# BoyBaykiller/IDKEngine

Measured on AMD Instinct MI355X. Metric: Mray/s (primary+1 bounce) at 1920x1080, 1M-tri scene, higher is better.
Workload: dtype f32

## Files before the change

### idkengine_amd/csrc/host_context.hpp

```cpp
#pragma once


struct DevBuf {
    void* p = nullptr; size_t bytes = 0;
    hipError_t ensure(size_t n) { if (n <= bytes && p) return hipSuccess; if (p) (void)hipFree(p); p = nullptr; bytes = 0; if (n == 0) return hipSuccess; hipError_t e = hipMalloc(&p, n); if (e == hipSuccess) bytes = n; return e; }
    void release() { if (p) (void)hipFree(p); p = nullptr; bytes = 0; }
    template <class T> T* as() const { return (T*)p; }
};

struct PinnedStage {
    char* host = nullptr; hipEvent_t ev[2] = {nullptr, nullptr}; int half = 0;
    template <class Fill> hipError_t stage(DevBuf& dst, size_t capacity, size_t bytes, hipStream_t st, Fill&& fill)
    {
        hipError_t e;
        if (!host) {
            if ((e = hipHostMalloc((void**)&host, 2 * capacity, hipHostMallocDefault)) != hipSuccess) return e;
            for (int i = 0; i < 2; i++) if ((e = hipEventCreateWithFlags(&ev[i], hipEventDisableTiming)) != hipSuccess) return e;
            half = 0;
        } else if ((e = hipEventSynchronize(ev[half])) != hipSuccess) return e;
        char* h = host + (size_t)half * capacity;
        fill(h);
        if ((e = dst.ensure(capacity)) != hipSuccess) return e;
        if ((e = hipMemcpyAsync(dst.p, h, bytes, hipMemcpyHostToDevice, st)) != hipSuccess) return e;
        if ((e = hipEventRecord(ev[half], st)) != hipSuccess) return e;
// ... 89 lines not shown
    void release() { if (host) (void)hipHostFree(host); host = nullptr; dev = nullptr; }
    template <class T> T* host_as() const { return (T*)host; }
    template <class T> T* dev_as() const { return (T*)dev; }
};
struct DerivedScene : derived::State {
    DevBuf wnodes, wleaf, wids, wpair, wcounts; std::vector<uint32_t> wNodeOff, wLeafOff;
    DevBuf pairNodes;
    DevBuf instRec;
    DevBuf itlas, imarks, ichunks; int itlasNeed = 1; uint32_t ichunkCount = 0;
    DevBuf entRec, braidBuf; bool itlasBraided = false; int itlasDepth = 0, itlasEntries = 0;
    MappedWords overlap; bool isieveWorth = false;
    int uniMode = 0; uint32_t uniBaseB = 0, uniRestoreIdx = 0;
    DevBuf unodes, utlas, uTabs, uniBuf, uniEntRec; bool uniEligible = false; int uniCap = 0, uniEntries = 0, uniDepth = 0; MappedWords uni;
    MappedWords pkStats; unsigned long long pkSeen[6] = {0, 0, 0, 0, 0, 0}; float pkCam[36] = {0}; int pkW = 0, pkRows = 0, pkBatch = 0; float pkLastLive = -1.0f;
    void release()
    {
        for (DevBuf* b : {&wnodes, &wleaf, &wids, &wpair, &wcounts, &pairNodes, &instRec, &itlas, &imarks, &ichunks, &entRec, &braidBuf, &unodes, &utlas, &uTabs, &uniBuf, &uniEntRec}) b->release();
        overlap.release(); uni.release(); pkStats.release(); valid = 0;
    }
};

struct DevOptions {
    int forceGeneric = 0;
    int noTileCull = 0;
    int noLeanPrimary = 0;
    int leafMin = 0;
    int grabUnitLog2 = 10, grabFixed = 0;
    int ldsPad = 0;
    int traceWaves = 0;
    int gridHint = 2;
    int deferLast = 1;
    int lastOcclusion = 1;
    int foldLast = 1;
    int graphProbe = 0;
    int gridMidWaves = 20;
    int gridRaysX4 = 6;
    int traceVariant = 0;
    int bvhTiming = 0, bvhSmall = 32;
    int advMin = 0;
    int poolMin = 12;
    int leafPool = -1;
    int splitScatter = 6;
    int queryScheduler = 1;
    int groupThreads = -1;
    int fused = 1;
    int fusedShadeMin = 16;
    int splitPeek = 64;
    int splitDonor = 1;
    int split = 1;
    int wide = 0;
    int wideCap = 0;
    int wideCount = 0;
    int genPixelMajor = 8;
    int bouncePixelMajor = 1;
    int genGroupMax = 16;
    int instSieve = 8;
    int instSieveOverlap = 50;
    int instTlas = 8;
    int instTlasOverlap = 10;
    int instBraid = 0;
    int instUnify = 4096;
    int instGeneral = 0;
    int uniRefill = 32;
    int instUnifyRadius = 15;
    int pairNodes = 1;
    int packet = 1;
// ... 34 lines not shown
    int sceneStack = 1;
    int hInst0Blas = 0;
    DerivedScene derived;
    DevBuf wtotals;
    std::vector<GpuBlasInstance> hInstances; std::vector<char> hXforms; uint64_t uniLaunches = 0;
    int verSlots = 1; size_t vbytes[VB_COUNT] = {0}, vstride[VB_COUNT] = {0}; int valloc[VB_COUNT] = {1, 1, 1, 1, 1}, vcur[VB_COUNT] = {0};
    uint64_t lastMask[VB_COUNT] = {0};
    uint8_t lastSlots[VB_COUNT] = {0}; bool lastMulti = false;
    DevBuf verTab; PinnedStage verStage;
    char* hStage = nullptr; hipEvent_t evStage[4] = {nullptr, nullptr, nullptr, nullptr}; int stageNext = 0;
    PinnedUpload skyStage;
    hipEvent_t evSky = nullptr;
    int (*groupFlushAll)(void* user) = nullptr;
    DevBuf pmList;
    DevBuf trRec, contFlag, blockSums, rayO, rayT, rayR, aovA, aovN, hit, hitCost, primHit, queue[2], keys[2], keysTmp, sortKeys, sortVals, contMask, waveCounts, counts, work, sortHist, counters64;
    DevBuf img[3];
    FrameProducts products;
    int presW = 0, presH = 0;
    int resultSource = 0;
    PinnedUpload denoiseStage;
    int denoiseInput = 0;
    DevBuf geomRays, geomHits;
    int noiseOn = 0;
    DevBuf camTab;
    int rowLimit = 0x7fffffff;
    idkpt_bounce_exchange_fn exchangeFn = nullptr; void* exchangeUser = nullptr;
    idkpt_band_exchange_fn bandExchangeFn = nullptr; void* bandExchangeUser = nullptr; DevBuf bandTab;
    idkpt_band_exchange_device_fn bandExchangeDevFn = nullptr; void* bandExchangeDevUser = nullptr;
    idkpt_stats stats;
    uint32_t* hCounts = nullptr; uint32_t* dCountsMirror = nullptr;
    bool sceneNested = false;
    bool sceneNoEmission = false;
    struct { bool valid = false, allHits = false; int j = 0, side = 0, B = 0; uint32_t total = 0, Npad = 0;
             bool occl = false, pm = false, fold = false; const uint32_t* list = nullptr; size_t ldsBytes = 0; uint32_t grid = 0; } defer;
    uint64_t occlLaunches = 0;
    uint64_t foldBatches = 0;
    DevBuf radSave, deferCount;
    bool countersDirty = true;
    uint32_t* hOverflow = nullptr; uint32_t* dOverflow = nullptr;
    int tlasNeed = 1;
    hipEvent_t evFrame[2] = {nullptr, nullptr};
    std::vector<hipEvent_t> evPool; size_t evUsed = 0;
    double traceMsAcc = 0.0; uint64_t traceLaunchesAcc = 0;
    int lastQueueSide = 0; int lastQueueCountSlot = 0; bool lastFast = false, lastNeedsRegen = false, lastTileClass = false ; int lastBatch = 1; Frame lastFrame;
    int maxBatch = 1; uint32_t Npad = 0; std::vector<PendingSample> pending; DevBuf bases, qwork; uint32_t* hBases = nullptr; uint32_t* dBasesMirror = nullptr;
    PinnedStage camStage;
    bool grouped = false, inGroupFlush = false; int groupIndex = 0;
    hipEvent_t* evBounce = nullptr;
    int (*groupExchange)(void* user, dev_ctx* member, int bounce, int samples, const uint32_t** outBases) = nullptr; void* groupUser = nullptr;
    struct BuilderScratch* bscratch = nullptr;
    struct PeerPolicy* peer = nullptr;
};

static hipEvent_t next_event(dev_ctx* ctx)
{
    if (ctx->evUsed == ctx->evPool.size()) { hipEvent_t e = nullptr; if (hipEventCreate(&e) != hipSuccess) return nullptr; ctx->evPool.push_back(e); }
    return ctx->evPool[ctx->evUsed++];
}
static void resolve_trace_events(dev_ctx* ctx)
{
    for (size_t i = 0; i + 1 < ctx->evUsed; i += 2) { float ms = 0.0f; if (hipEventElapsedTime(&ms, ctx->evPool[i], ctx->evPool[i + 1]) == hipSuccess) { ctx->traceMsAcc += ms; ctx->traceLaunchesAcc++; } }
    ctx->evUsed = 0;
}
#define TRACE_T0() do { if (ctx->timing) { hipEvent_t _e = next_event(ctx); if (_e) (void)hipEventRecord(_e, st); } } while (0)
#define TRACE_T1() do { if (ctx->timing) { hipEvent_t _e = next_event(ctx); if (_e) (void)hipEventRecord(_e, st); } } while (0)

static int fail(dev_ctx* c, int code, const std::string& msg) { if (c) { c->lastError = msg; if (c->errFn) c->errFn(c->errUser, (int32_t)code, c->lastError.c_str()); } return code; }
#define HIPC(expr) do { hipError_t _e = (expr); if (_e != hipSuccess) { (void)hipGetLastError(); return fail(ctx, IDKPT_ERR_HIP, std::string(#expr) + ": " + hipGetErrorString(_e)); } } while (0)
#define REQUIRE(cond, msg) do { if (!(cond)) return fail(ctx, IDKPT_ERR_INVALID_ARGUMENT, msg); } while (0)
// ... 26 lines not shown
```

### idkengine_amd/csrc/host_options.hpp

```cpp
#pragma once

static int32_t dev_SetOption(dev_ctx* ctx, const char* name, int32_t value)
{
    if (!ctx || !name) return IDKPT_ERR_INVALID_ARGUMENT;
    HIPC(hipSetDevice(ctx->device));
    FLUSH();
    DevOptions& o = ctx->opt;
    const std::string n(name);
    if (n == "force_generic") o.forceGeneric = value != 0;
    else if (n == "no_tile_cull") o.noTileCull = value != 0;
    else if (n == "no_lean_primary") o.noLeanPrimary = value != 0;
    else if (n == "leaf_min") o.leafMin = std::max(0, value);
    else if (n == "grab_unit_log2") o.grabUnitLog2 = value;
    else if (n == "grab_fixed") o.grabFixed = value;
    else if (n == "lds_pad") o.ldsPad = value;
    else if (n == "trace_waves") o.traceWaves = std::max(0, value);
    else if (n == "grid_hint") o.gridHint = std::max(0, value);
    else if (n == "grid_rays_x4") o.gridRaysX4 = std::max(0, value);
    else if (n == "grid_mid_waves") o.gridMidWaves = std::max(0, value);
    else if (n == "defer_last") o.deferLast = value != 0;
    else if (n == "last_occlusion") o.lastOcclusion = value != 0;
    else if (n == "fold_last") o.foldLast = value != 0;
    else if (n == "split") { REQUIRE(value >= 0 && value <= 3, "idkptSetDeveloperOption: split is 0..3"); o.split = value; }
    else if (n == "split_donor") o.splitDonor = value != 0;
    else if (n == "split_peek") o.splitPeek = std::max(1, value);
    else if (n == "split_scatter") o.splitScatter = std::min(6, std::max(0, value));
    else if (n == "query_scheduler") o.queryScheduler = value != 0;
    else if (n == "group_threads") o.groupThreads = value;
    else if (n == "fused") { REQUIRE(value >= 0 && value <= 2, "idkptSetDeveloperOption: fused is 0..2"); o.fused = value; }
    else if (n == "fused_shade_min") o.fusedShadeMin = std::min(64, std::max(1, value));
    else if (n == "leaf_pool") { REQUIRE(value >= -1 && value <= 7, "idkptSetDeveloperOption: leaf_pool is -1 (automatic) or a mask 0..7 (1: primary launches, 2: the first bounce, 4: later bounces)"); o.leafPool = value; }
    else if (n == "pool_min") o.poolMin = std::max(0, value);
    else if (n == "adv_min") o.advMin = std::min(64, std::max(0, value));
#ifdef IDKPT_DEVELOPER
    else if (n == "graph_probe") o.graphProbe = std::max(0, value);
#endif
    else if (n == "inst_tlas_overlap") { REQUIRE(value >= 0 && value <= 100, "idkptSetDeveloperOption: inst_tlas_overlap is a percentage"); FLUSH(); o.instTlasOverlap = value; ctx->derived.invalidate(derived::Cause::InstOption); }
    else if (n == "bounce_pixel_major") { REQUIRE(value >= 0 && value <= 2, "idkptSetDeveloperOption: bounce_pixel_major is 0..2"); o.bouncePixelMajor = value; }
    else if (n == "gen_group_max") { REQUIRE(value >= 1 && value <= 16, "idkptSetDeveloperOption: gen_group_max is 1..16"); o.genGroupMax = value; }
    else if (n == "gen_pixel_major") { REQUIRE(value >= 0, "idkptSetDeveloperOption: gen_pixel_major is >= 0"); o.genPixelMajor = value; }
    else if (n == "inst_sieve_overlap") { REQUIRE(value >= 0 && value <= 100, "idkptSetDeveloperOption: inst_sieve_overlap is a percentage"); FLUSH(); o.instSieveOverlap = value; ctx->derived.invalidate(derived::Cause::InstOption); }
    else if (n == "inst_sieve") { REQUIRE(value >= 0, "idkptSetDeveloperOption: inst_sieve is >= 0"); FLUSH(); o.instSieve = value; ctx->derived.invalidate(derived::Cause::InstOption); }
    else if (n == "inst_braid") { REQUIRE(value >= 0, "idkptSetDeveloperOption: inst_braid is >= 0"); FLUSH(); o.instBraid = value; ctx->derived.invalidate(derived::Cause::InstOption); }
    else if (n == "pair_nodes") { REQUIRE(value == 0 || value == 1, "idkptSetDeveloperOption: pair_nodes is 0 or 1"); o.pairNodes = value; }
    else if (n == "inst_general") { REQUIRE(value >= 0, "idkptSetDeveloperOption: inst_general is >= 0"); FLUSH(); o.instGeneral = value; ctx->derived.invalidate(derived::Cause::InstOption); }
    else if (n == "uni_refill") { REQUIRE(value == 16 || value == 32, "idkptSetDeveloperOption: uni_refill is 16 or 32"); o.uniRefill = value; }
    else if (n == "inst_unify_radius") { REQUIRE(value >= 1 && value <= 512, "idkptSetDeveloperOption: inst_unify_radius is 1-512"); FLUSH(); o.instUnifyRadius = value; ctx->derived.invalidate(derived::Cause::InstOption); }
    else if (n == "inst_unify") { REQUIRE(value >= 0, "idkptSetDeveloperOption: inst_unify is >= 0"); FLUSH(); o.instUnify = value; ctx->derived.invalidate(derived::Cause::InstOption); }
    else if (n == "inst_tlas") { REQUIRE(value >= 0, "idkptSetDeveloperOption: inst_tlas is >= 0"); FLUSH(); o.instTlas = value; ctx->derived.invalidate(derived::Cause::InstOption); }
    else if (n == "packet") { REQUIRE(value >= 0 && value <= 2, "idkptSetDeveloperOption: packet is 0..2"); o.packet = value; ctx->derived.packet_reprobe(); }
    else if (n == "packet_min_live") { REQUIRE(value >= 0 && value <= 100, "idkptSetDeveloperOption: packet_min_live is a percentage"); o.packetMinLive = value; ctx->derived.packet_reprobe(); }
    else if (n == "packet_waves") { REQUIRE(value >= 0 && value <= 32, "idkptSetDeveloperOption: packet_waves is 0 (default) or 1..32"); o.packetWaves = value; }
    else if (n == "wide") { REQUIRE(value >= 0 && value <= 1, "idkptSetDeveloperOption: wide is 0 or 1"); FLUSH(); o.wide = value; }
    else if (n == "wide_cap") { REQUIRE(value >= 0 && value <= 96, "idkptSetDeveloperOption: wide_cap is 0 (default) or 4..96 rows"); o.wideCap = value; }
    else if (n == "wide_count") o.wideCount = value != 0;
// ... 15 lines not shown
```

### idkengine_amd/csrc/host_readback.hpp

```cpp
#pragma once

static int32_t dev_DownloadFrame(dev_ctx* ctx, int32_t slot, int32_t image, float* rgba, size_t bytes)
{
    if (!ctx || !rgba) return IDKPT_ERR_INVALID_ARGUMENT;
    REQUIRE(image >= 0 && image < 3, "idkptDownloadFrame: bad image id");
    REQUIRE(slot >= 0 && slot < ctx->ringSize, "idkptDownloadFrame: slot outside the frame ring");
    size_t need = (size_t)ctx->W * ctx->rows * 16;
    REQUIRE(bytes == need && need > 0, "idkptDownloadFrame: bytes must equal localRows*width*16");
    HIPC(hipSetDevice(ctx->device));
    FLUSH_KEEP();
    HIPC(hipMemcpyAsync(rgba, image_ptr(ctx, image, slot), need, hipMemcpyDeviceToHost, ctx->stream));
    SYNC_CHECKED();
    return IDKPT_OK;
}

static int32_t dev_GetFrameDevicePtr(dev_ctx* ctx, int32_t slot, int32_t image, void** outPtr, size_t* outBytes)
{
    if (!ctx || !outPtr) return IDKPT_ERR_INVALID_ARGUMENT;
    REQUIRE(image >= 0 && image < 3, "idkptGetFrameDevicePtr: bad image id");
    REQUIRE(slot >= 0 && slot < ctx->ringSize, "idkptGetFrameDevicePtr: slot outside the frame ring");
    HIPC(hipSetDevice(ctx->device));
    FLUSH_KEEP();
    { int rc = check_overflow(ctx); if (rc) return rc; }
    *outPtr = image_ptr(ctx, image, slot);
// ... 80 lines not shown
    const bool have = ctx->lastFast && ctx->lastTileClass;
    const int32_t tx = have ? (ctx->lastFrame.W + 7) / 8 : 0, ty = have ? (ctx->lastFrame.rows + 7) / 8 : 0;
    const int32_t n = have ? (ctx->lastFrame.tilePerSample ? ctx->lastBatch : 1) : 0;
    *tilesX = tx; *tilesY = ty; *sets = n;
    if (!out) return IDKPT_OK;
    const size_t need = (size_t)n * tx * ty;
    REQUIRE(bytes == need, "idkptDownloadTileClasses: bytes must equal sets*tilesX*tilesY (call with out = NULL for the three numbers)");
    if (need) { REQUIRE(ctx->tileClass.bytes >= need, "idkptDownloadTileClasses: no classification is resident"); HIPC(hipMemcpyAsync(out, ctx->tileClass.p, need, hipMemcpyDeviceToHost, ctx->stream)); }
    SYNC_CHECKED();
    return IDKPT_OK;
}

static int32_t dev_GetStats(dev_ctx* ctx, idkpt_stats* out)
{
    if (!ctx || !out) return IDKPT_ERR_INVALID_ARGUMENT;
    HIPC(hipSetDevice(ctx->device));
    FLUSH_KEEP();
    SYNC_CHECKED();
    idkpt_stats s = ctx->stats;
    for (int j = 0; j < 16; j++) { const uint32_t* hb = ctx->hBases + (size_t)j * (MAX_BATCH + 1); s.LastAliveCounts[j] = (j >= 1 && j < ctx->st.RayDepth) ? hb[ctx->lastBatch] - hb[ctx->lastBatch - 1] : 0; }
    s.LastAliveCounts[0] = s.Frames ? (ctx->lastFast ? ctx->hCounts[MAX_DEPTH_SLOTS - 1] : (uint32_t)((size_t)ctx->W * ctx->rows)) : 0;
    s.LastFrameMs = 0.0f; s.LastTraceMs = 0.0f;
    if (ctx->timing && s.Frames > 0) { float ms = 0.0f; if (hipEventElapsedTime(&ms, ctx->evFrame[0], ctx->evFrame[1]) == hipSuccess) s.LastFrameMs = ms; }
    resolve_trace_events(ctx);
    s.TraceMsTotal = ctx->traceMsAcc; s.TraceLaunches = ctx->traceLaunchesAcc;
    s.LastTraceMs = s.TraceLaunches ? (float)(s.TraceMsTotal / (double)s.TraceLaunches) : 0.0f;
    uint64_t c[4] = {0, 0, 0, 0};
    HIPC(hipMemcpyAsync(c, ctx->counters64.p, 32, hipMemcpyDeviceToHost, ctx->stream)); HIPC(hipStreamSynchronize(ctx->stream));
    s.NodePairVisits = c[0]; s.TriangleTests = c[1];
    if (ctx->opt.traceVariant == 107 || ctx->opt.traceVariant == 113 || ctx->opt.traceVariant == 116 || ctx->opt.traceVariant == 213) { uint64_t d[16]; HIPC(hipMemcpyAsync(d, ctx->counters64.p, 128, hipMemcpyDeviceToHost, ctx->stream)); HIPC(hipStreamSynchronize(ctx->stream)); fprintf(stderr, "[idkpt prof] cycles refill %llu node %llu leaf %llu other %llu | refills %llu lanes %llu | nodeSteps %llu lanes %llu | leafPhases %llu lanes %llu | leafTests %llu leafTrips %llu\n", (unsigned long long)d[4], (unsigned long long)d[5], (unsigned long long)d[6], (unsigned long long)d[7], (unsigned long long)d[8], (unsigned long long)d[9], (unsigned long long)d[10], (unsigned long long)d[11], (unsigned long long)d[12], (unsigned long long)d[13], (unsigned long long)d[14], (unsigned long long)d[15]); }
    s.RaysTraced = s.PrimaryRays + c[2];
    if (ctx->wtotals.p) { uint64_t w[16]; HIPC(hipMemcpyAsync(w, ctx->wtotals.p, TOTALS_BYTES, hipMemcpyDeviceToHost, ctx->stream)); HIPC(hipStreamSynchronize(ctx->stream)); s.WideFlaggedRays = w[0]; s.WideNodeVisits = w[1]; s.WideLeafRecords = w[2]; s.WideTriangleTests = w[3]; s.InstTlasFlaggedRays = w[4];
        s.PacketFlaggedRays = w[8]; s.PacketPackets = w[9]; s.PacketNodeSteps = w[10]; s.PacketLiveLanes = w[11]; s.PacketRaysEntered = w[12]; s.PacketTriangleRounds = w[13]; }
    s.LastOcclusionLaunches = ctx->occlLaunches; s.LastFoldBatches = ctx->foldBatches;
    s.InstUnifiedLaunches = ctx->uniLaunches; s.InstUnifiedEntries = ctx->derived.holds(derived::UNI) ? (uint32_t)ctx->derived.uniEntries : 0u; s.InstUnifiedTopDepth = ctx->derived.holds(derived::UNI) ? (uint32_t)ctx->derived.uniDepth : 0u;
    *out = s;
    return IDKPT_OK;
}

static int32_t dev_ResetStats(dev_ctx* ctx)
{
    if (!ctx) return IDKPT_ERR_INVALID_ARGUMENT;
    HIPC(hipSetDevice(ctx->device));
    FLUSH_KEEP();
    HIPC(hipStreamSynchronize(ctx->stream));
    memset(&ctx->stats, 0, sizeof(ctx->stats)); ctx->uniLaunches = 0; ctx->occlLaunches = 0; ctx->foldBatches = 0;
    if (ctx->derived.pkStats.host) memset(ctx->derived.pkStats.host, 0, 64);
    for (int i = 0; i < 6; i++) ctx->derived.pkSeen[i] = 0;
    ctx->evUsed = 0; ctx->traceMsAcc = 0.0; ctx->traceLaunchesAcc = 0;
    memset(ctx->hCounts, 0, (MAX_DEPTH_SLOTS - 1) * 4);
    HIPC(hipMemsetAsync(ctx->counters64.p, 0, 128, ctx->stream)); if (ctx->wtotals.p) HIPC(hipMemsetAsync(ctx->wtotals.p, 0, TOTALS_BYTES, ctx->stream)); HIPC(hipStreamSynchronize(ctx->stream));
    return IDKPT_OK;
}

static int32_t dev_EnableCounters(dev_ctx* ctx, int32_t enable) { if (!ctx) return IDKPT_ERR_INVALID_ARGUMENT; ctx->counters = enable != 0; return IDKPT_OK; }
static int32_t dev_EnableTiming(dev_ctx* ctx, int32_t enable) { if (!ctx) return IDKPT_ERR_INVALID_ARGUMENT; ctx->timing = enable != 0; return IDKPT_OK; }

static int32_t dev_GetImageDevicePtr(dev_ctx* ctx, int32_t image, void** outPtr, size_t* outBytes)
{
    if (!ctx || !outPtr) return IDKPT_ERR_INVALID_ARGUMENT;
    REQUIRE(image >= 0 && image < 3 && ctx->W > 0, "idkptGetImageDevicePtr: bad image / no size");
    HIPC(hipSetDevice(ctx->device));
    FLUSH_KEEP();
    { int rc = check_overflow(ctx); if (rc) return rc; }
    *outPtr = image_ptr(ctx, image, ctx->curSlot);
    if (outBytes) *outBytes = (size_t)ctx->W * ctx->rows * 16;
    return IDKPT_OK;
}

static int32_t dev_SetStream(dev_ctx* ctx, void* hipStream)
{
    if (!ctx) return IDKPT_ERR_INVALID_ARGUMENT;
    HIPC(hipSetDevice(ctx->device));
    FLUSH();
    HIPC(hipStreamSynchronize(ctx->stream));
    if (hipStream) { if (ctx->ownStream && ctx->stream) (void)hipStreamDestroy(ctx->stream); ctx->stream = (hipStream_t)hipStream; ctx->ownStream = false; }
    else if (!ctx->ownStream) { HIPC(hipStreamCreateWithFlags(&ctx->stream, hipStreamNonBlocking)); ctx->ownStream = true; }
    return IDKPT_OK;
}
// ... 83 lines not shown
```

### idkengine_amd/csrc/host_schedule.hpp

```cpp
#pragma once

static DScene make_dscene(dev_ctx* ctx, const uint8_t* slots, bool multi)
{
    DScene s;
    auto at = [&](int b) -> char* { return multi ? (char*)vb_buf(ctx, b).p : vb_ptr(ctx, b, slots ? slots[b] : ctx->vcur[b]); };
    s.nodes = (const float4*)at(VB_NODES); s.tris = ctx->tris.as<uint4>(); s.triVerts = (const float4*)at(VB_TRIVERTS);
    s.descs = ctx->descs.as<GpuBlasDesc>(); s.instances = ctx->instances.as<GpuBlasInstance>(); s.instanceCount = ctx->instanceCount;
    s.tlas = (const float4*)at(VB_TLAS); s.tlasCount = ctx->tlasCount; s.vertices = (const uint4*)at(VB_VERTICES);
    s.instRec = nullptr;
    s.pairNodes = nullptr;
    s.meshes = ctx->meshes.as<GpuMesh>(); s.materials = ctx->materials.as<GpuMaterial>(); s.xforms = (const float4*)at(VB_XFORMS);
    s.lights = ctx->lights.as<GpuLight>(); s.lightCount = ctx->lightCount; s.sky = ctx->sky.as<float4>(); s.skySize = ctx->skySize;
    s.textures = ctx->texDescs.as<TexDesc>(); s.textureCount = ctx->textureCount; s.srgbLut = ctx->srgbLut.as<float>();
    s.overflow = ctx->dOverflow;
    s.ver = multi ? ctx->verTab.as<uint32_t>() : nullptr;
    return s;
}
static DScene make_dscene(dev_ctx* ctx) { return make_dscene(ctx, nullptr, false); }
static DScene make_dscene_last(dev_ctx* ctx) { return make_dscene(ctx, ctx->lastSlots, ctx->lastMulti); }

static float4* image_ptr(dev_ctx* ctx, int i, int slot) { return ctx->img[i].as<float4>() + (size_t)slot * ((size_t)ctx->W * ctx->rows); }

#define GRID_MID_RAYS 14000000u
#define SPLIT_MAX_RAYS 1500000u
static bool want_split(const dev_ctx* ctx, uint32_t prev, bool known, int samples)
{
    if (ctx->opt.split == 0) return false;
    if (ctx->opt.split >= 2) return true;
    return known && sparse_view(ctx, samples) && prev > 0u && prev < SPLIT_MAX_RAYS;
}
#define FUSED_MAX_RAYS 600000u
static bool want_fused(const dev_ctx* ctx, uint32_t prev, bool known, int samples)
{
    if (ctx->opt.fused == 0) return false;
    if (ctx->opt.fused >= 2) return true;
    return known && prev > 0u && prev < FUSED_MAX_RAYS && few_traversed(ctx, prev, std::max(1, samples));
}
static bool want_occlusion(const dev_ctx* ctx, const TracePlan& plan, bool readsOnlyHitOrMiss, bool split)
{
    return readsOnlyHitOrMiss && ctx->opt.lastOcclusion != 0 && !plan.fused && (plan.walk == Walk::Plain || plan.walk == Walk::Fast) && !(split && plan.splitOk)
           && !plan.multiVer && !plan.counting && !ctx->counters && (ctx->opt.traceVariant == 0 || ctx->opt.traceVariant == 100);
}
static bool want_fold(const dev_ctx* ctx, bool tookOccl) { return tookOccl && ctx->opt.foldLast != 0; }
static bool may_fold(const dev_ctx* ctx, bool deferLast, bool deferAllHits) { return deferLast && !deferAllHits && ctx->opt.lastOcclusion != 0 && ctx->opt.foldLast != 0; }
static uint32_t small_launch_grid(uint32_t fullGrid, uint32_t prev, int hintMul, int raysX4, uint32_t midGrid)
{
    if (prev == 0u || hintMul <= 0) return fullGrid;
    const uint32_t cap = std::max<uint32_t>(256u, (uint32_t)(((uint64_t)hintMul * prev + 63) / 64));
    uint32_t g = cap;
    if (raysX4 > 0) g = std::max<uint32_t>((uint32_t)(((uint64_t)prev * 4u / (uint32_t)raysX4 + 63) / 64), std::min<uint32_t>(cap, 1024u));
    if (midGrid > 0u && prev < GRID_MID_RAYS) g = std::min(g, midGrid);
    return std::min(fullGrid, std::min(g, cap));
}

struct Batch {
    dev_ctx* ctx; hipStream_t st; int B, depth; uint32_t N, Npad, total, gridTotal, scanBlocks;
    bool multiVer, fast, debug, capturing;
    Frame f; DScene s; TracePlan plan;
    RayBufs rays; HitBufs hits; TraceBufs tr, trNone;
    uint32_t* counts; uint32_t* bases ; uint32_t* work; uint64_t* counters; uint32_t* hostCounts; uint32_t* hostBases;
    unsigned long long* contMask; uint32_t* waveLocal ; uint32_t* blockSums; uint32_t* keysTmp;
    uint32_t* activeList; uint32_t* activeCount;
    uint32_t* pmList; uint32_t* pmCount; bool pmBounce;
    const uint8_t* tileClass; uint32_t midGrid, traceGrid;
    int side;
};
static const int BS = MAX_BATCH + 1;

static void batch_views(dev_ctx* ctx, Batch& b, int B, uint32_t Npad)
{
    b.ctx = ctx; b.st = ctx->stream; b.B = B; b.depth = ctx->st.RayDepth; b.N = (uint32_t)((size_t)ctx->W * ctx->rows); b.Npad = Npad; b.total = (uint32_t)B * Npad;
    b.gridTotal = (b.total + 255) / 256; b.scanBlocks = ((b.total + 63) / 64 + SCAN_WAVES_PER_BLOCK - 1) / SCAN_WAVES_PER_BLOCK;
    b.rays = {ctx->rayO.as<float4>(), ctx->rayT.as<float4>(), ctx->rayR.as<float4>(), ctx->aovA.as<float4>(), ctx->aovN.as<float4>(), ctx->contFlag.as<uint8_t>()}; b.hits = {ctx->hit.as<float4>(), ctx->hitCost.as<float>()};
    b.tr = {ctx->trRec.as<float4>(), nullptr, nullptr, ctx->deferCount.as<uint32_t>() + 1}; b.trNone = {nullptr, nullptr, nullptr, nullptr};
    b.counts = ctx->counts.as<uint32_t>(); b.bases = ctx->bases.as<uint32_t>(); b.work = ctx->work.as<uint32_t>(); b.counters = ctx->counters64.as<uint64_t>(); b.hostCounts = ctx->dCountsMirror; b.hostBases = ctx->dBasesMirror;
    b.contMask = ctx->contMask.as<unsigned long long>(); b.waveLocal = ctx->waveCounts.as<uint32_t>(); b.blockSums = ctx->blockSums.as<uint32_t>(); b.keysTmp = ctx->keysTmp.as<uint32_t>();
    b.activeList = ctx->sortVals.as<uint32_t>(); b.activeCount = b.counts + (MAX_DEPTH_SLOTS - 1);
    b.pmList = nullptr; b.pmCount = b.counts + (MAX_DEPTH_SLOTS - 2); b.pmBounce = false; b.tileClass = nullptr; b.side = 1; b.capturing = false;
}

static int bounce_tail(Batch& b, int j, const uint32_t* q, const uint32_t* cnt, const uint32_t* gbase, unsigned long long* traced, bool record, const TraceBufs& tr)
{
    dev_ctx* ctx = b.ctx; hipStream_t st = b.st; const int side = b.side;
    with_flag(b.multiVer, [&](auto VER) { launch(k_shade<false, VER>, dim3(b.gridTotal), dim3(256), 0, st, b.s, b.f, b.rays, tr, b.hits, q, cnt, 0u, b.bases + j * BS, gbase, b.contMask, b.waveLocal, b.keysTmp); });
    launch(k_scan_local<false>, dim3(b.scanBlocks), dim3(SCAN_WAVES_PER_BLOCK), 0, st, cnt, 0u, nullptr, b.contMask, b.waveLocal, b.blockSums);
    launch(k_scan_blocks, dim3(1), dim3(1024), 0, st, cnt, 0u, b.blockSums, b.waveLocal, b.counts + j + 1, traced, b.contMask, b.bases + j * BS, b.Npad, b.B, b.bases + (j + 1) * BS, b.hostCounts + j + 1, b.hostBases + (size_t)(j + 1) * BS, nullptr, nullptr);
    if (record) HIPC(hipEventRecord(ctx->evBounce[j + 1], st));
    launch(k_compact<false>, dim3(b.gridTotal), dim3(256), 0, st, q, cnt, 0u, b.contMask, b.waveLocal, b.blockSums, b.keysTmp, ctx->queue[1 - side].as<uint32_t>(), ctx->keys[1 - side].as<uint32_t>());
    return IDKPT_OK;
}

static int finish_deferred(dev_ctx* ctx)
{
    if (!ctx->defer.valid) return IDKPT_OK;
    ctx->defer.valid = false;
    Batch b; batch_views(ctx, b, ctx->defer.B, ctx->defer.Npad);
    b.side = ctx->defer.side; b.f = ctx->lastFrame; b.f.markLast = 0; b.f.foldLast = 0; b.s = make_dscene_last(ctx); b.multiVer = ctx->lastMulti;
    const uint32_t* q = ctx->queue[b.side].as<uint32_t>(); const uint32_t* cnt = ctx->deferCount.as<uint32_t>();
    if (ctx->defer.occl) {
        const int j = ctx->defer.j;
        if (ctx->countersDirty) HIPC(hipMemsetAsync(b.work, 0, WORK_WORDS * 4, b.st));
        TracePlan p{}; p.walk = Walk::Plain; p.ldsBytes = ctx->defer.ldsBytes; p.grid = ctx->defer.grid;
        Frame ft = b.f; if (ctx->defer.pm) ft.hitsByRid = 0;
        if (ctx->defer.pm) launch_trace2<true>(ctx, p, p.grid, b.st, b.s, ft, b.rays, b.tr, b.hits, ctx->defer.list, cnt, b.work + j, b.counters, false, j);
        else launch_trace2<false>(ctx, p, p.grid, b.st, b.s, ft, b.rays, b.tr, b.hits, q, cnt, b.work + j, b.counters, false, j);
        ctx->defer.occl = false;
    }
    with_flag(ctx->defer.allHits, [&](auto ALL) { launch(k_restore_last<ALL>, dim3(b.gridTotal), dim3(256), 0, b.st, b.rays, b.hits, q, cnt, ctx->radSave.as<float4>(), b.f.hitsByRid, ctx->defer.fold ? 1 : 0); });
    { int rc = bounce_tail(b, ctx->defer.j, q, cnt, nullptr, nullptr, false, b.tr); if (rc) return rc; }
    HIPC(hipGetLastError());
    ctx->lastQueueSide = 1 - b.side; ctx->countersDirty = true;
    return IDKPT_OK;
}

static int stage_versions_cameras(Batch& b)
{
    dev_ctx* ctx = b.ctx; const int B = b.B;
    bool multiVer = false; for (int k = 1; k < B && !multiVer; k++) multiVer = memcmp(ctx->pending[k].vs, ctx->pending[0].vs, VB_COUNT) != 0;
    for (int v = 0; v < VB_COUNT; v++) { uint64_t m = 0; for (int k = 0; k < B; k++) m |= 1ull << ctx->pending[k].vs[v]; ctx->lastMask[v] = m; ctx->lastSlots[v] = ctx->pending[0].vs[v]; }
    ctx->lastMulti = b.multiVer = multiVer;
    auto fillVersions = [&](char* half) {
        for (int k = 0; k < B; k++) {
            const uint8_t* vs = ctx->pending[k].vs; uint32_t* row = (uint32_t*)half + (size_t)k * SCENE_VER_WORDS;
            for (int v = 0; v < VB_COUNT; v++) row[v] = (uint32_t)(((size_t)vs[v] * ctx->vstride[v]) / 16);
            for (int v = VB_COUNT; v < SCENE_VER_WORDS; v++) row[v] = 0u;
        } };
    if (multiVer) HIPC(ctx->verStage.stage(ctx->verTab, (size_t)MAX_BATCH * SCENE_VER_WORDS * 4, (size_t)B * SCENE_VER_WORDS * 4, b.st, fillVersions));
    b.s = make_dscene_last(ctx);
    memset(&b.f, 0, sizeof(b.f));
    if (ctx->ringSize > 1) {
        auto fillCameras = [&](char* half) { for (int k = 0; k < B; k++) memcpy(half + (size_t)k * 36 * 4, ctx->pending[k].cam, 36 * 4); };
// ... 5 lines not shown

#ifdef IDKPT_DEVELOPER
static void graph_probe_begin(Batch& b) { if (b.ctx->opt.graphProbe > 0 && !b.ctx->timing) b.capturing = hipStreamBeginCapture(b.st, hipStreamCaptureModeThreadLocal) == hipSuccess; }
static void graph_probe_end(Batch& b)
{
    if (!b.capturing) return;
    dev_ctx* ctx = b.ctx; hipStream_t st = b.st;
    hipGraph_t g = nullptr; hipGraphExec_t ex = nullptr; const int K = ctx->opt.graphProbe; ctx->opt.graphProbe = 0;
    if (hipStreamEndCapture(st, &g) == hipSuccess && g && hipGraphInstantiate(&ex, g, nullptr, nullptr, 0) == hipSuccess) {
        hipEvent_t e0 = nullptr, e1 = nullptr; (void)hipEventCreate(&e0); (void)hipEventCreate(&e1);
        (void)hipGraphLaunch(ex, st); (void)hipStreamSynchronize(st);
        (void)hipEventRecord(e0, st);
        for (int k = 0; k < K; k++) (void)hipGraphLaunch(ex, st);
        (void)hipEventRecord(e1, st); (void)hipStreamSynchronize(st);
        float ms = 0.0f; (void)hipEventElapsedTime(&ms, e0, e1);
        size_t nodes = 0; (void)hipGraphGetNodes(g, nullptr, &nodes);
        fprintf(stderr, "[idkpt graph] batch of %d sample(s) captured: %zu graph nodes; %d replays: %.1f us per batch\n", b.B, nodes, K, ms * 1000.0f / (float)K);
        (void)hipEventDestroy(e0); (void)hipEventDestroy(e1); (void)hipGraphExecDestroy(ex);
    } else fprintf(stderr, "[idkpt graph] capture or instantiation failed: %s\n", hipGetErrorString(hipGetLastError()));
    if (g) (void)hipGraphDestroy(g);
}
#else
static void graph_probe_begin(Batch&) {}
static void graph_probe_end(Batch&) {}
#endif

static int frame_setup(Batch& b)
{
    dev_ctx* ctx = b.ctx; hipStream_t st = b.st; Frame& f = b.f; const int B = b.B;
    memcpy(f.invProj, ctx->pending[0].cam, 64); memcpy(f.invView, ctx->pending[0].cam + 16, 64); memcpy(f.viewPos, ctx->pending[0].cam + 32, 12);
    f.W = ctx->W; f.H = ctx->H; f.rowMod = ctx->rowMod; f.rowRem = ctx->rowRem; f.rows = ctx->rows; f.rowBandLog2 = ctx->rowBandLog2;
    f.g = ctx->st.Gpu; f.useTlas = ctx->st.UseTlas; f.stackCap = std::max(1, ctx->st.BlasStackSize > 0 ? ctx->st.BlasStackSize : ctx->sceneStack);
    f.outputAovs = ctx->st.OutputAOVs; f.batch = B; f.Npad = b.Npad;
    HIPC(ctx->trRec.ensure((size_t)ctx->maxBatch * b.Npad * 64)); b.tr.rec = ctx->trRec.as<float4>();
    for (int k = 0; k < MAX_BATCH; k++) { f.accum[k] = k < B ? ctx->pending[k].accum : 0u; f.slotOf[k] = (uint32_t)(k < B ? ctx->pending[k].slot : 0); }
    f.seqFirst = ctx->seqFirst; f.seqStride = ctx->seqStride; f.accumulated = f.seqFirst + f.accum[0] * f.seqStride;
    f.tilePerSample = (f.cams != nullptr || b.multiVer) ? 1 : 0;
    graph_probe_begin(b);
    if (ctx->timing) HIPC(hipEventRecord(ctx->evFrame[0], st));
    ctx->defer.valid = false;
    if (ctx->countersDirty) { HIPC(hipMemsetAsync(b.work, 0, WORK_WORDS * 4, st)); HIPC(hipMemsetAsync(b.counts, 0, MAX_DEPTH_SLOTS * 4, st)); HIPC(hipMemsetAsync(b.tr.oddCount, 0, 4, st)); }
    ctx->countersDirty = true;
    f.tlasCap = std::min(TLAS_STACK_SIZE, std::max(1, ctx->tlasNeed));
    f.grabUnitLog2 = std::min(24, std::max(6, ctx->opt.grabUnitLog2)); f.grabFixed = std::max(0, ctx->opt.grabFixed);
    f.leafMin = ctx->opt.leafMin > 0 ? ctx->opt.leafMin : (B >= 4 ? 16 : 12);
    b.fast = fast_path(ctx);
    f.genPixelMajor = (b.fast && ctx->opt.genPixelMajor > 0 && B >= ctx->opt.genPixelMajor && !f.tilePerSample) ? 1 : 0;
    { int rc = trace_plan(ctx, f, b.s, b.multiVer, false, false, b.plan); if (rc) { ctx->pending.clear(); return rc; } }
    b.traceGrid = std::min<uint32_t>(b.plan.grid, std::max<uint32_t>(1u, (uint32_t)(((size_t)B * b.N + 63) / 64)));
    b.midGrid = (ctx->opt.gridMidWaves > 0 && ctx->opt.traceWaves == 0) ? (uint32_t)(ctx->numCUs * std::min(b.plan.wavesPerCU, ctx->opt.gridMidWaves)) : 0u;
    f.gridRaysX4 = (uint32_t)std::max(0, ctx->opt.gridRaysX4); f.gridMid = b.midGrid; f.gridMidRays = GRID_MID_RAYS; f.splitMode = (ctx->opt.split == 3 ? 2 : 1) | (ctx->opt.splitDonor ? 4 : 0); f.poolMin = ctx->opt.poolMin; f.advMin = ctx->opt.advMin > 0 ? ctx->opt.advMin : (B >= 4 ? 8 : 1); f.splitPeek = ctx->opt.splitPeek;
    b.debug = f.g.DoDebugBVHTraversal != 0; f.shadeMin = ctx->opt.fusedShadeMin; f.scatterLog2 = ctx->opt.splitScatter;
    if (!b.fast && (B != 1 || b.multiVer)) { ctx->pending.clear(); return fail(ctx, IDKPT_ERR_UNKNOWN, "internal: generic path is never batched"); }
    return IDKPT_OK;
}

static int first_hit_compact(Batch& b)
{
    dev_ctx* ctx = b.ctx; hipStream_t st = b.st;
    launch(k_scan_blocks, dim3(1), dim3(1024), 0, st, nullptr, b.total, b.blockSums, b.waveLocal, b.counts + 1, (unsigned long long*)(1 < b.depth ? b.counters + 2 : nullptr), b.contMask, nullptr, b.Npad, b.B, b.bases + 1 * BS, b.hostCounts + 1, b.hostBases + 1 * BS, b.counts + MAX_DEPTH_SLOTS - 1, b.hostCounts + MAX_DEPTH_SLOTS - 1);
    if (ctx->evBounce) HIPC(hipEventRecord(ctx->evBounce[1], st));
    launch(k_compact<true>, dim3(b.gridTotal), dim3(256), 0, st, nullptr, nullptr, b.total, b.contMask, b.waveLocal, b.blockSums, b.keysTmp, ctx->queue[1].as<uint32_t>(), ctx->keys[1].as<uint32_t>());
    return IDKPT_OK;
}

static int first_hit_fast(Batch& b)
{
    dev_ctx* ctx = b.ctx; hipStream_t st = b.st; Frame& f = b.f; const DScene& s = b.s; const int B = b.B; const uint32_t N = b.N;
    const uint32_t tilesX = ((uint32_t)f.W + 7) / 8, tilesY = ((uint32_t)f.rows + 7) / 8; const uint32_t genWaves = tilesX * tilesY;
    const int cull = f.g.DoTraceLights ? 0 : 1;
    const int lean = (cull && !f.useTlas && s.instanceCount == 1 && ctx->opt.noLeanPrimary == 0) ? 1 : 0;
    uint8_t* contFlag = ctx->contFlag.as<uint8_t>();
    if (ctx->capturePrimary) launch(k_fill_miss, dim3((N + 255) / 256), dim3(256), 0, st, b.hits, (size_t)(B - 1) * b.Npad, N);
    if (cull && !ctx->opt.noTileCull) {
        const uint32_t classSets = f.tilePerSample ? (uint32_t)B : 1u;
        HIPC(ctx->tileClass.ensure((size_t)genWaves * classSets));
        with_flag(b.multiVer, [&](auto VER) { launch(k_classify_tiles<VER>, dim3((genWaves + 255) / 256, classSets), dim3(256), 0, st, s, f, ctx->tileClass.as<uint8_t>(), tilesX, tilesY); });
        b.tileClass = ctx->tileClass.as<uint8_t>();
    }
    const int genMax = std::min(16, std::max(1, ctx->opt.genGroupMax)), genGroups = (B + genMax - 1) / genMax, genPer = (B + genGroups - 1) / genGroups;
    const dim3 genGrid = f.genPixelMajor ? dim3(genGroups, genWaves) : dim3(B, (genWaves + 15) / 16), genBlock = f.genPixelMajor ? dim3(64 * genPer) : dim3(1024);
    with_flag(b.multiVer, [&](auto VER) { launch(k_gen_primary<VER>, genGrid, genBlock, 0, st, s, f, b.rays, b.tr, cull, b.activeList, b.activeCount, b.keysTmp, contFlag, b.tileClass, lean); });
    TRACE_T0();
    const bool known = ctx->lastFast && ctx->lastBatch == B;
    uint32_t grid0 = b.traceGrid;
    if (ctx->opt.gridRaysX4 > 0 && known) grid0 = small_launch_grid(b.traceGrid, ctx->hCounts[MAX_DEPTH_SLOTS - 1], 2, ctx->opt.gridRaysX4, b.midGrid);
    if (b.plan.fused) launch(k_trace_fused<32>, dim3(grid0), dim3(WAVE), b.plan.ldsBytes, st, s, f, b.rays, b.tr, b.hits, b.activeList, b.activeCount, b.work + 0, contFlag, b.keysTmp, lean);
    else launch_trace2<true>(ctx, b.plan, grid0, st, s, f, b.rays, b.tr, b.hits, b.activeList, b.activeCount, b.work + 0, b.counters, want_split(ctx, ctx->hCounts[MAX_DEPTH_SLOTS - 1], known, B), 0);
    TRACE_T1();
    if (ctx->capturePrimary) { HIPC(ctx->primHit.ensure((size_t)N * 16)); launch(k_capture_primary, dim3((N + 255) / 256), dim3(256), 0, st, b.hits, (size_t)(B - 1) * b.Npad, N, ctx->primHit.as<float4>()); }
    if (!b.plan.fused) {
        const bool sparseView = ctx->lastFast && ctx->lastBatch >= 1 && few_traversed(ctx, ctx->hCounts[MAX_DEPTH_SLOTS - 1], ctx->lastBatch);
        b.pmBounce = f.genPixelMajor && (ctx->opt.bouncePixelMajor >= 2 || (ctx->opt.bouncePixelMajor == 1 && sparseView)) && b.depth >= 2 && !b.multiVer;
        if (b.pmBounce) { HIPC(ctx->pmList.ensure((size_t)b.total * 4)); b.pmList = ctx->pmList.as<uint32_t>(); }
        with_flag(b.multiVer, [&](auto VER) { launch(k_shade_first<VER>, dim3(b.gridTotal), dim3(256), 0, st, s, f, b.rays, b.tr, b.hits, b.activeList, b.activeCount, contFlag, b.keysTmp, lean, b.pmList, VER ? nullptr : b.pmCount); });
    }
    launch(k_scan_local<true>, dim3(b.scanBlocks), dim3(SCAN_WAVES_PER_BLOCK), 0, st, nullptr, b.total, contFlag, b.contMask, b.waveLocal, b.blockSums);
    return first_hit_compact(b);
}

static int first_hit_generic(Batch& b)
{
    dev_ctx* ctx = b.ctx; hipStream_t st = b.st; const uint32_t N = b.N;
    TRACE_T0();
    const uint32_t g = std::min<uint32_t>(b.traceGrid, (N + 63) / 64);
    with_flags(ctx->counters, b.debug, [&](auto COUNT, auto COST) { launch(k_trace_primary<COUNT, COST>, dim3(g), dim3(WAVE), b.plan.ldsBytes, st, b.s, b.f, b.rays, b.hits, N, b.work + 0, b.counters); });
    TRACE_T1();
    if (ctx->capturePrimary) { HIPC(ctx->primHit.ensure((size_t)N * 16)); launch(k_capture_primary, dim3((N + 255) / 256), dim3(256), 0, st, b.hits, 0, N, ctx->primHit.as<float4>()); }
    launch(k_shade<true, false>, dim3(b.gridTotal), dim3(256), 0, st, b.s, b.f, b.rays, b.trNone, b.hits, nullptr, nullptr, b.total, nullptr, nullptr, b.contMask, b.waveLocal, b.keysTmp);
    launch(k_scan_local<false>, dim3(b.scanBlocks), dim3(SCAN_WAVES_PER_BLOCK), 0, st, nullptr, b.total, nullptr, b.contMask, b.waveLocal, b.blockSums);
    return first_hit_compact(b);
}

static int exchange_bases(Batch& b, int j, const uint32_t* q, const uint32_t*& gbase)
{
    dev_ctx* ctx = b.ctx; hipStream_t st = b.st; Frame& f = b.f; const int B = b.B;
    gbase = nullptr; f.gbStride = 1; f.gbBands = 0;
    const bool bandExchange = (ctx->bandExchangeFn || ctx->bandExchangeDevFn) && ctx->rowMod > 1 && !(ctx->st.DoRaySorting && j > 1);
    if (!bandExchange && ctx->groupExchange) {
        const int rc = ctx->groupExchange(ctx->groupUser, ctx, j, B, &gbase); if (rc) ctx->pending.clear(); return rc; }
    if (!bandExchange && ctx->exchangeFn) {
        std::vector<uint32_t> hb(B + 1), local(B), outBases(B, 0u);
        HIPC(hipMemcpyAsync(hb.data(), b.bases + j * BS, (size_t)(B + 1) * 4, hipMemcpyDeviceToHost, st)); HIPC(hipStreamSynchronize(st));
        for (int b2 = 0; b2 < B; b2++) local[b2] = hb[b2 + 1] - hb[b2];
        ctx->exchangeFn(ctx->exchangeUser, j, B, local.data(), outBases.data());
        HIPC(ctx->gbases.ensure((size_t)MAX_BATCH * 4));
        HIPC(hipMemcpyAsync(ctx->gbases.p, outBases.data(), (size_t)B * 4, hipMemcpyHostToDevice, st)); HIPC(hipStreamSynchronize(st));
        gbase = ctx->gbases.as<uint32_t>();
    }
// ... 12 lines not shown
    } else {
        std::vector<uint32_t> starts((size_t)B * (LB + 1)), local((size_t)B * LB), outBases((size_t)B * LB, 0u), tab((size_t)B * LB);
        HIPC(hipMemcpyAsync(starts.data(), dStarts, starts.size() * 4, hipMemcpyDeviceToHost, st)); HIPC(hipStreamSynchronize(st));
        for (int k2 = 0; k2 < B; k2++) for (int b2 = 0; b2 < LB; b2++) local[(size_t)k2 * LB + b2] = starts[(size_t)k2 * (LB + 1) + b2 + 1] - starts[(size_t)k2 * (LB + 1) + b2];
        ctx->bandExchangeFn(ctx->bandExchangeUser, j, B, LB, local.data(), outBases.data());
        for (int k2 = 0; k2 < B; k2++) for (int b2 = 0; b2 < LB; b2++) tab[(size_t)k2 * LB + b2] = outBases[(size_t)k2 * LB + b2] - starts[(size_t)k2 * (LB + 1) + b2];
        HIPC(hipMemcpyAsync(dTab, tab.data(), tab.size() * 4, hipMemcpyHostToDevice, st)); HIPC(hipStreamSynchronize(st));
    }
    gbase = dTab; f.gbStride = LB; f.gbBands = 1;
    return IDKPT_OK;
}

static int sort_queue(Batch& b, uint32_t* q, uint32_t* k, const uint32_t* cnt)
{
    dev_ctx* ctx = b.ctx; hipStream_t st = b.st;
    const uint32_t nTiles = (b.total + SORT_TILE - 1) / SORT_TILE;
    int sampleBits = 0; while ((1 << sampleBits) < b.B) sampleBits++;
    const int passes = (IDKPT_SORT_KEY_BITS + sampleBits + 6) / 7;
    uint32_t* hist = ctx->sortHist.as<uint32_t>(); uint32_t* digitTotals = hist + (size_t)SORT_RADIX * nTiles;
    uint32_t* ka = k; uint32_t* va = q; uint32_t* kb = ctx->sortKeys.as<uint32_t>(); uint32_t* vb = ctx->sortVals.as<uint32_t>();
    for (int pass = 0; pass < passes; pass++) {
        launch(k_sort_hist, dim3(nTiles), dim3(SORT_BLOCK), 0, st, ka, cnt, (uint32_t)(7 * pass), hist, nTiles);
        launch(k_sort_scan, dim3(SORT_RADIX), dim3(1024), 0, st, cnt, hist, nTiles, digitTotals);
        launch(k_sort_scatter, dim3(nTiles), dim3(SORT_BLOCK), 0, st, ka, va, cnt, (uint32_t)(7 * pass), hist, nTiles, digitTotals, kb, vb);
        std::swap(ka, kb); std::swap(va, vb);
    }
    if (va != q) HIPC(hipMemcpyAsync(q, va, (size_t)b.total * 4, hipMemcpyDeviceToDevice, st));
    return IDKPT_OK;
}

static bool trace_bounce(Batch& b, int j, const uint32_t* q, const uint32_t* cnt, bool readsOnlyHitOrMiss)
{
    dev_ctx* ctx = b.ctx; hipStream_t st = b.st; const int B = b.B;
    TRACE_T0();
    const bool known = ctx->lastFast && ctx->lastBatch == B && ctx->hBases != nullptr; const uint32_t prev = ctx->hBases ? ctx->hBases[(size_t)j * BS + B] : 0u;
    uint32_t gridj = b.traceGrid;
    const bool split = want_split(ctx, prev, known, B), occl = b.fast && want_occlusion(ctx, b.plan, readsOnlyHitOrMiss, split);
    if (occl) ctx->occlLaunches++;
    if (want_fold(ctx, occl)) { b.f.foldLast = 1; b.f.hitsByRid = 1; }
    if (ctx->opt.gridHint > 0 && ctx->lastBatch == B && ctx->hBases) gridj = small_launch_grid(b.traceGrid, ctx->hBases[(size_t)j * BS + B], ctx->opt.gridHint, ctx->opt.gridRaysX4, b.midGrid);
    if (b.fast && ((b.pmBounce && j == 1) || b.f.foldLast)) {
        const bool pm = b.pmBounce && j == 1;
        Frame ft = b.f; ft.hitsByRid = 0;
        launch_trace2<true>(ctx, b.plan, gridj, st, b.s, ft, b.rays, b.tr, b.hits, pm ? b.pmList : q, pm ? b.pmCount : cnt, b.work + j, b.counters, split, j, occl);
    } else if (b.fast) launch_trace2<false>(ctx, b.plan, gridj, st, b.s, b.f, b.rays, b.tr, b.hits, q, cnt, b.work + j, b.counters, split, j, occl);
    else with_flag(ctx->counters, [&](auto COUNT) { launch(k_trace_queue<COUNT>, dim3(b.traceGrid), dim3(WAVE), b.plan.ldsBytes, st, b.s, b.f, b.rays, b.hits, q, cnt, b.work + j, b.counters); });
    TRACE_T1();
    return occl;
}

static int defer_last_bounce(Batch& b, int j, const uint32_t* q, const uint32_t* cnt, bool allHits, bool occl)
{
    dev_ctx* ctx = b.ctx;
    const bool fold = b.f.foldLast != 0, pm = b.pmBounce && j == 1;
    HIPC(ctx->radSave.ensure((size_t)ctx->maxBatch * ctx->Npad * 16));
    auto shade_last = [&](auto ALL, auto VER) { launch(k_shade_last<ALL, VER>, dim3(b.gridTotal), dim3(256), 0, b.st, b.s, b.f, b.rays, b.hits, q, cnt, b.bases + j * BS, ctx->radSave.as<float4>(), ctx->deferCount.as<uint32_t>()); };
    if (fold) launch(k_shade_last_odd, dim3(std::min<uint32_t>(b.gridTotal, 256u)), dim3(256), 0, b.st, b.s, b.f, b.rays, b.hits, q, cnt, b.bases + j * BS, ctx->radSave.as<float4>(), ctx->deferCount.as<uint32_t>(), (const uint32_t*)b.tr.oddCount);
    else if (allHits) with_flag(b.multiVer, [&](auto VER) { shade_last(std::true_type{}, VER); });
    else shade_last(std::false_type{}, std::false_type{});
    if (fold) ctx->foldBatches++;
    ctx->defer.allHits = allHits; ctx->defer.valid = true; ctx->defer.j = j; ctx->defer.side = b.side; ctx->defer.B = b.B; ctx->defer.total = b.total; ctx->defer.Npad = b.Npad;
    ctx->defer.occl = occl; ctx->defer.fold = fold; ctx->defer.pm = pm || fold; ctx->defer.list = pm ? (const uint32_t*)b.pmList : q; ctx->defer.ldsBytes = b.plan.ldsBytes; ctx->defer.grid = b.traceGrid;
    return IDKPT_OK;
}

static int final_draw(Batch& b)
{
    dev_ctx* ctx = b.ctx; hipStream_t st = b.st;
    ctx->lastQueueSide = b.side; ctx->lastQueueCountSlot = b.depth; ctx->lastFast = b.fast; ctx->lastNeedsRegen = b.fast; ctx->lastTileClass = b.tileClass != nullptr; ctx->lastBatch = b.B; ctx->lastFrame = b.f;
    if (ctx->noiseOn) {
        launch(k_final_draw_noise, dim3((b.N + 255) / 256), dim3(256), 0, st, b.s, b.f, b.rays, image_ptr(ctx, 0, 0), image_ptr(ctx, 1, 0), image_ptr(ctx, 2, 0), b.N, b.tileClass, b.work, (uint32_t)WORK_WORDS, b.counts, (uint32_t)MAX_DEPTH_SLOTS, b.tr.oddCount,
               noise_moments_ptr(ctx, 0), noise_mom_stride(ctx));
    } else
    launch(k_final_draw, dim3((b.N + 255) / 256), dim3(256), 0, st, b.s, b.f, b.rays, image_ptr(ctx, 0, 0), image_ptr(ctx, 1, 0), image_ptr(ctx, 2, 0), b.N, b.tileClass, b.work, (uint32_t)WORK_WORDS, b.counts, (uint32_t)MAX_DEPTH_SLOTS, b.tr.oddCount);
    HIPC(hipGetLastError()); ctx->countersDirty = false;
    graph_probe_end(b);
    if (ctx->timing) HIPC(hipEventRecord(ctx->evFrame[1], st));
    ctx->stats.Frames += (uint64_t)b.B; ctx->stats.PrimaryRays += (uint64_t)b.N * (uint64_t)b.B;
    ctx->pending.clear();
    return IDKPT_OK;
}

static int flush_batch(dev_ctx* ctx)
{
    if (ctx->pending.empty()) return IDKPT_OK;
    if (ctx->grouped && !ctx->inGroupFlush) return fail(ctx, IDKPT_ERR_UNKNOWN, "internal: a member of a multi-device context was flushed on its own");
    if (ctx->noiseOn) { int rc = noise_moments_ensure(ctx); if (rc) return rc; }
    Batch b; batch_views(ctx, b, (int)ctx->pending.size(), ctx->Npad); int rc;
    if ((rc = stage_versions_cameras(b))) return rc;
    if ((rc = frame_setup(b))) return rc;
    const bool deferLast = b.fast && b.depth >= 2 && ctx->opt.deferLast != 0 && !b.f.outputAovs && !b.debug;
    const bool deferAllHits = !(ctx->sceneNoEmission && !(b.f.g.DoTraceLights && b.s.lightCount > 0));
    const bool mayFold = may_fold(ctx, deferLast, deferAllHits);
// ... 109 lines not shown
```

### idkengine_amd/csrc/idkpt_api.hpp

```cpp
#pragma once
#include <array>
#include <thread>
#include <mutex>
#include <condition_variable>
#include <functional>

struct GroupBarrier {
    std::mutex m; std::condition_variable cv; int n = 0, arrived = 0; unsigned gen = 0; bool aborted = false;
    void reset(int members) { std::lock_guard<std::mutex> l(m); n = members; arrived = 0; aborted = false; }
    bool wait()
    {
        std::unique_lock<std::mutex> l(m);
        if (aborted) return false;
        const unsigned g = gen;
        if (++arrived == n) { arrived = 0; gen++; cv.notify_all(); return true; }
        cv.wait(l, [&] { return gen != g || aborted; });
        return !aborted;
    }
    void abort() { std::lock_guard<std::mutex> l(m); aborted = true; cv.notify_all(); }
};
struct GroupWorkers {
    std::vector<std::thread> th;
    std::mutex m; std::condition_variable cvGo, cvDone;
    unsigned epoch = 0; int remaining = 0; bool quit = false;
// ... 941 lines not shown
    ONE(dev_DownloadTileClasses(m, out, bytes, tilesX, tilesY, sets));
    GFLUSH();
    dev_ctx* m = c->dev[0];
    const int rc = dev_DownloadTileClasses(m, out, bytes, tilesX, tilesY, sets);
    return rc ? mfail(c, m, rc) : IDKPT_OK;
}
int32_t idkptDownloadPrimaryHits(idkpt_ctx* c, float* t, uint32_t* triangleId, float* baryXY, size_t pixelCount)
{
    if (!c || !t || !triangleId || !baryXY) return IDKPT_ERR_INVALID_ARGUMENT;
    ONE(dev_DownloadPrimaryHits(m, t, triangleId, baryXY, pixelCount));
    GREQ(pixelCount == (size_t)c->W * c->H, "idkptDownloadPrimaryHits: pixelCount mismatch");
    GFLUSH();
    for (size_t d = 0; d < c->n(); d++) {
        dev_ctx* m = c->dev[d];
        const size_t N = (size_t)c->W * m->rows;
        std::vector<float> tt(N), bb(2 * N); std::vector<uint32_t> ii(N);
        int rc = dev_DownloadPrimaryHits(m, tt.data(), ii.data(), bb.data(), N); if (rc) return mfail(c, m, rc);
        for (size_t i = 0; i < N; i++) { const uint32_t g = global_pixel(c, (int)d, (uint32_t)i); t[g] = tt[i]; triangleId[g] = ii[i]; baryXY[2 * (size_t)g] = bb[2 * i]; baryXY[2 * (size_t)g + 1] = bb[2 * i + 1]; }
    }
    return IDKPT_OK;
}

int32_t idkptGetStats(idkpt_ctx* c, idkpt_stats* out)
{
    if (!c || !out) return IDKPT_ERR_INVALID_ARGUMENT;
    ONE(dev_GetStats(m, out));
    GFLUSH();
    idkpt_stats sum; memset(&sum, 0, sizeof(sum));
    for (size_t d = 0; d < c->n(); d++) {
        idkpt_stats s; int rc = dev_GetStats(c->dev[d], &s); if (rc) return mfail(c, c->dev[d], rc);
        sum.RaysTraced += s.RaysTraced; sum.PrimaryRays += s.PrimaryRays; sum.NodePairVisits += s.NodePairVisits; sum.TriangleTests += s.TriangleTests;
        sum.WideFlaggedRays += s.WideFlaggedRays; sum.WideNodeVisits += s.WideNodeVisits; sum.WideLeafRecords += s.WideLeafRecords; sum.WideTriangleTests += s.WideTriangleTests; sum.InstTlasFlaggedRays += s.InstTlasFlaggedRays;
        sum.PacketFlaggedRays += s.PacketFlaggedRays; sum.PacketPackets += s.PacketPackets; sum.PacketNodeSteps += s.PacketNodeSteps; sum.PacketLiveLanes += s.PacketLiveLanes; sum.PacketRaysEntered += s.PacketRaysEntered; sum.PacketTriangleRounds += s.PacketTriangleRounds;
        sum.LastOcclusionLaunches += s.LastOcclusionLaunches; sum.LastFoldBatches += s.LastFoldBatches;
        sum.InstUnifiedLaunches += s.InstUnifiedLaunches; if (d == 0) { sum.InstUnifiedEntries = s.InstUnifiedEntries; sum.InstUnifiedTopDepth = s.InstUnifiedTopDepth; }
        for (int j = 0; j < 16; j++) sum.LastAliveCounts[j] += s.LastAliveCounts[j];
        sum.LastFrameMs = std::max(sum.LastFrameMs, s.LastFrameMs); sum.LastTraceMs = std::max(sum.LastTraceMs, s.LastTraceMs);
        sum.TraceMsTotal = std::max(sum.TraceMsTotal, s.TraceMsTotal);
        if (d == 0) { sum.Frames = s.Frames; sum.TraceLaunches = s.TraceLaunches; }
    }
    *out = sum;
    return IDKPT_OK;
}
int32_t idkptGetStatsSized(idkpt_ctx* c, void* out, size_t bytes)
{
    if (!c || !out) return IDKPT_ERR_INVALID_ARGUMENT;
    idkpt_stats s; const int32_t rc = idkptGetStats(c, &s); if (rc) return rc;
    memcpy(out, &s, std::min(bytes, sizeof(s)));
    return IDKPT_OK;
}
int32_t idkptResetStats(idkpt_ctx* c) { REPLICATE(ResetStats); }
int32_t idkptEnableCounters(idkpt_ctx* c, int32_t enable) { if (!c) return IDKPT_ERR_INVALID_ARGUMENT; ONE(dev_EnableCounters(m, enable)); GFLUSH(); for (dev_ctx* m : c->dev) dev_EnableCounters(m, enable); return IDKPT_OK; }
int32_t idkptEnableTiming(idkpt_ctx* c, int32_t enable) { if (!c) return IDKPT_ERR_INVALID_ARGUMENT; for (dev_ctx* m : c->dev) dev_EnableTiming(m, enable); return IDKPT_OK; }

int32_t idkptSetStream(idkpt_ctx* c, void* hipStream)
{
    if (!c) return IDKPT_ERR_INVALID_ARGUMENT;
    ONE(dev_SetStream(m, hipStream));
    return gfail(c, IDKPT_ERR_INVALID_OPERATION, "idkptSetStream: a multi-device context owns one stream per device");
}
int32_t idkptGetStream(idkpt_ctx* c, void** out) { if (!c || !out) return IDKPT_ERR_INVALID_ARGUMENT; return dev_GetStream(c->dev[0], out); }

}
```

### idkengine_amd/csrc/kernels_frame.hpp

```cpp
#pragma once
#include "noise_texel.hpp"

DEV f3 TurboColormap(float x)
{
    x = gclamp(x, 0.0f, 1.0f);
    float v0 = 1.0f, v1 = x, v2 = x * x, v3 = x * x * x;
    float w0 = v2 * v2, w1 = v3 * v2;
    float r = (((v0 * 0.13572138f + v1 * 4.61539260f) + v2 * -42.66032258f) + v3 * 132.13108234f) + (w0 * -152.94239396f + w1 * 59.28637943f);
    float g = (((v0 * 0.09140261f + v1 * 2.19418839f) + v2 * 4.84296658f) + v3 * -14.18503333f) + (w0 * 4.27729857f + w1 * 2.82956604f);
    float b = (((v0 * 0.10667330f + v1 * 12.64194608f) + v2 * -60.58204836f) + v3 * 110.36276771f) + (w0 * -89.90310912f + w1 * 27.34824973f);
    return mk3(r, g, b);
}
template <bool NOISE>
__device__ __forceinline__ void final_draw_body(const DScene& s, const Frame& f, const RayBufs& rays, float4* imgResult, float4* imgAlbedo, float4* imgNormal, uint32_t N, const uint8_t* tileClass,
                                                uint32_t i, float4* imgMoments, size_t momStride)
{
    uint32_t slot = f.slotOf[0];
    float4 o = imgResult[(size_t)slot * N + i];
    f3 r = mk3(o.x, o.y, o.z), ra = splat3(0.0f), rn = splat3(0.0f);
    if (f.outputAovs) { float4 oa = imgAlbedo[(size_t)slot * N + i], on = imgNormal[(size_t)slot * N + i]; ra = mk3(oa.x, oa.y, oa.z); rn = mk3(on.x, on.y, on.z); }
    float m1 = 0.0f, m2 = 0.0f;
    if constexpr (NOISE) { const float4 om = imgMoments[(size_t)slot * momStride + i]; m1 = om.x; m2 = om.y; }
    const uint32_t px = i % (uint32_t)f.W, py = i / (uint32_t)f.W, tilesX = ((uint32_t)f.W + 7) / 8;
    const uint32_t tile = (py >> 3) * tilesX + (px >> 3), nTilesAll = tilesX * (((uint32_t)f.rows + 7) / 8);
    const uint32_t sharedCls = (tileClass && !f.tilePerSample) ? tileClass[tile] : 0u;
    for (int k = 0; k < f.batch; k++) {
        if (f.slotOf[k] != slot) {
            imgResult[(size_t)slot * N + i] = make_float4(r.x, r.y, r.z, 1.0f);
            if (f.outputAovs) { imgAlbedo[(size_t)slot * N + i] = make_float4(ra.x, ra.y, ra.z, 1.0f); imgNormal[(size_t)slot * N + i] = make_float4(rn.x, rn.y, rn.z, 1.0f); }
            if constexpr (NOISE) imgMoments[(size_t)slot * momStride + i] = make_float4(m1, m2, 0.0f, 1.0f);
            slot = f.slotOf[k];
            o = imgResult[(size_t)slot * N + i]; r = mk3(o.x, o.y, o.z);
            if (f.outputAovs) { float4 oa = imgAlbedo[(size_t)slot * N + i], on = imgNormal[(size_t)slot * N + i]; ra = mk3(oa.x, oa.y, oa.z); rn = mk3(on.x, on.y, on.z); }
            if constexpr (NOISE) { const float4 om = imgMoments[(size_t)slot * momStride + i]; m1 = om.x; m2 = om.y; }
        }
        const size_t rid = (size_t)k * f.Npad + i;
        float w = 1.0f / ((float)f.accum[k] + 1.0f);
        const uint32_t cls = !tileClass ? 0u : (f.tilePerSample ? tileClass[(size_t)k * nTilesAll + tile] : sharedCls);
        f3 nr = splat3(0.0f);
        if (cls == 0u) {
            const float4 c = rays.rad_py[rid]; nr = mk3(c.x, c.y, c.z);
            if (f.foldLast && (rays.flag[rid] & CF_LAST_MISSED)) {
                const float4 b = rays.thr_px[rid];
                if (__builtin_isfinite(b.x) && __builtin_isfinite(b.y) && __builtin_isfinite(b.z)) {
                    const f3 albedo = SampleSky(s, DecodeUnitVec(b.w, c.w));
                    nr = mk3(c.x, c.y, c.z) + albedo * mk3(b.x, b.y, b.z);
                }
            }
        }
        else if (cls <= 6u) { const float4 p = s.sky[cls - 1u]; nr = splat3(0.0f) + mk3(p.x, p.y, p.z) * splat3(1.0f); }
        else if (cls == 8u) {
            f3 origin; f2 pd; uint32_t seed;
            gen_primary(f, (uint32_t)k, i, sample_index(f, (uint32_t)k), origin, pd, seed);
            const f3 albedo = SampleSky(s, DecodeUnitVec(pd.x, pd.y));
            nr = splat3(0.0f) + albedo * splat3(1.0f);
        }
        if (f.g.DoDebugBVHTraversal) nr = TurboColormap(rays.o_ior[rid].w / 150.0f);
        r = gmix(r, nr, w);
        if constexpr (NOISE) noiset::fold(&m1, &m2, noiset::luminance(nr.x, nr.y, nr.z), w);
        if (f.outputAovs) { float4 a = rays.aovA[rid], n = rays.aovN[rid]; ra = gmix(ra, mk3(a.x, a.y, a.z), w); rn = gmix(rn, mk3(n.x, n.y, n.z), w); }
    }
    imgResult[(size_t)slot * N + i] = make_float4(r.x, r.y, r.z, 1.0f);
    if (f.outputAovs) { imgAlbedo[(size_t)slot * N + i] = make_float4(ra.x, ra.y, ra.z, 1.0f); imgNormal[(size_t)slot * N + i] = make_float4(rn.x, rn.y, rn.z, 1.0f); }
    if constexpr (NOISE) imgMoments[(size_t)slot * momStride + i] = make_float4(m1, m2, 0.0f, 1.0f);
}
__global__ __launch_bounds__(256) void k_final_draw(DScene s, Frame f, RayBufs rays, float4* imgResult, float4* imgAlbedo, float4* imgNormal, uint32_t N, const uint8_t* tileClass,
                                                    uint32_t* zeroWork, uint32_t nWork, uint32_t* zeroCounts, uint32_t nCounts, uint32_t* zeroOdd )
{
    if (blockIdx.x == 0) { for (uint32_t k = threadIdx.x; k < nWork; k += blockDim.x) zeroWork[k] = 0u; for (uint32_t k = threadIdx.x; k < nCounts; k += blockDim.x) zeroCounts[k] = 0u; if (threadIdx.x == 0) *zeroOdd = 0u; }
    uint32_t i = blockIdx.x * blockDim.x + threadIdx.x;
    if (i >= N) return;
    final_draw_body<false>(s, f, rays, imgResult, imgAlbedo, imgNormal, N, tileClass, i, nullptr, 0);
}
__global__ __launch_bounds__(256) void k_final_draw_noise(DScene s, Frame f, RayBufs rays, float4* imgResult, float4* imgAlbedo, float4* imgNormal, uint32_t N, const uint8_t* tileClass,
                                                          uint32_t* zeroWork, uint32_t nWork, uint32_t* zeroCounts, uint32_t nCounts, uint32_t* zeroOdd, float4* imgMoments, size_t momStride)
{
    if (blockIdx.x == 0) { for (uint32_t k = threadIdx.x; k < nWork; k += blockDim.x) zeroWork[k] = 0u; for (uint32_t k = threadIdx.x; k < nCounts; k += blockDim.x) zeroCounts[k] = 0u; if (threadIdx.x == 0) *zeroOdd = 0u; }
    uint32_t i = blockIdx.x * blockDim.x + threadIdx.x;
    if (i >= N) return;
    final_draw_body<true>(s, f, rays, imgResult, imgAlbedo, imgNormal, N, tileClass, i, imgMoments, momStride);
}

__global__ __launch_bounds__(256) void k_regen_culled(DScene s, Frame f, RayBufs rays, const uint8_t* contFlag, const uint8_t* tileClass, uint32_t smp, uint32_t N)
{
    const uint32_t pix = blockIdx.x * blockDim.x + threadIdx.x;
    if (pix >= N) return;
    const size_t rid = (size_t)smp * f.Npad + pix;
    uint8_t flag = contFlag[rid];
    if (tileClass) {
        const uint32_t px = pix % (uint32_t)f.W, py = pix / (uint32_t)f.W, tilesX = ((uint32_t)f.W + 7) / 8, nTilesAll = tilesX * (((uint32_t)f.rows + 7) / 8);
        if (tileClass[(f.tilePerSample ? (size_t)smp * nTilesAll : 0) + (py >> 3) * tilesX + (px >> 3)] != 0u) flag = CF_CULLED_TILE;
    }
    flag &= (uint8_t)(CF_CULLED_PIXEL | CF_CULLED_TILE);
    if (flag == 0) return;
    f3 origin; f2 pd; uint32_t seed;
    gen_primary(f, smp, pix, sample_index(f, smp), origin, pd, seed);
    rays.o_ior[rid] = make_float4(origin.x, origin.y, origin.z, 1.0f);
    rays.thr_px[rid] = make_float4(1.0f, 1.0f, 1.0f, pd.x);
    if (flag == CF_CULLED_TILE) {
        const f3 albedo = SampleSky(s, DecodeUnitVec(pd.x, pd.y));
        const f3 radiance = splat3(0.0f) + albedo * splat3(1.0f);
        rays.rad_py[rid] = make_float4(radiance.x, radiance.y, radiance.z, pd.y);
    }
}

__global__ void k_fill_miss(HitBufs hits, size_t first, uint32_t n)
{
    uint32_t i = blockIdx.x * blockDim.x + threadIdx.x;
    if (i < n) store_hit(hits, first + i, PT_FLOAT_MAX, 0.0f, 0.0f, ~0u, 0u);
}

__global__ void k_gather_triverts(const uint4* tris, const float* positions, float4* triVerts, uint32_t first, uint32_t count)
{
    uint32_t i = blockIdx.x * blockDim.x + threadIdx.x;
    if (i >= count) return;
    uint4 t = tris[first + i];
    const float* a = positions + 3 * (size_t)t.x; const float* b = positions + 3 * (size_t)t.y; const float* c = positions + 3 * (size_t)t.z;
    float4* o = triVerts + 3 * (size_t)(first + i);
    o[0] = make_float4(a[0], a[1], a[2], 0.0f); o[1] = make_float4(b[0], b[1], b[2], 0.0f); o[2] = make_float4(c[0], c[1], c[2], 0.0f);
}

__global__ void k_capture_primary(HitBufs hits, size_t first, uint32_t n, float4* out)
{
    uint32_t i = blockIdx.x * blockDim.x + threadIdx.x;
    if (i < n) out[i] = hits.hit[2 * (first + i)];
}
```

### idkengine_amd/csrc/kernels_queue.hpp

```cpp
#pragma once

__global__ __launch_bounds__(256) void k_band_counts(const uint32_t* starts, int B, int LB, uint32_t* counts)
{
    const uint32_t t = blockIdx.x * blockDim.x + threadIdx.x;
    if (t >= (uint32_t)B * (uint32_t)LB) return;
    const uint32_t k = t / (uint32_t)LB, b = t % (uint32_t)LB;
    counts[t] = starts[k * (uint32_t)(LB + 1) + b + 1] - starts[k * (uint32_t)(LB + 1) + b];
}
__global__ __launch_bounds__(256) void k_band_tab(const uint32_t* starts, const uint32_t* bases, int B, int LB, uint32_t* tab)
{
    const uint32_t t = blockIdx.x * blockDim.x + threadIdx.x;
    if (t >= (uint32_t)B * (uint32_t)LB) return;
    const uint32_t k = t / (uint32_t)LB, b = t % (uint32_t)LB;
    tab[t] = bases[t] - starts[k * (uint32_t)(LB + 1) + b];
}

__global__ __launch_bounds__(256) void k_band_starts(const uint32_t* queue, const uint32_t* bases, int B, int LB, uint32_t bandPixels, uint32_t Npad, uint32_t* starts)
{
    const uint32_t t = blockIdx.x * blockDim.x + threadIdx.x;
    if (t >= (uint32_t)B * (uint32_t)(LB + 1)) return;
    const uint32_t k = t / (uint32_t)(LB + 1), b = t % (uint32_t)(LB + 1);
    const uint32_t lo0 = bases[k], hi0 = bases[k + 1];
    const unsigned long long key = (unsigned long long)k * Npad + (unsigned long long)b * bandPixels;
    uint32_t lo = lo0, hi = hi0;
    while (lo < hi) { const uint32_t mid = lo + ((hi - lo) >> 1); if ((unsigned long long)queue[mid] < key) lo = mid + 1; else hi = mid; }
    starts[t] = lo - lo0;
}

#define SCAN_WAVES_PER_BLOCK 256
template <bool FROM_FLAGS>
__global__ __launch_bounds__(SCAN_WAVES_PER_BLOCK) void k_scan_local(const uint32_t* countPtr, uint32_t countImm, uint8_t* contFlag, unsigned long long* contMask, uint32_t* waveLocal, uint32_t* blockSums)
{
    __shared__ uint32_t part[SCAN_WAVES_PER_BLOCK];
    const uint32_t N = countPtr ? *countPtr : countImm;
    const uint32_t nW = (N + 63) / 64;
    const uint32_t w = blockIdx.x * SCAN_WAVES_PER_BLOCK + threadIdx.x;
    if (blockIdx.x * SCAN_WAVES_PER_BLOCK >= nW) return;
    uint32_t c = 0;
    if (w < nW) {
        unsigned long long m;
        if (FROM_FLAGS) {
            uint4* p = reinterpret_cast<uint4*>(contFlag + (size_t)w * 64);
            m = 0ull;
            for (int q = 0; q < 4; q++) {
                uint4 v = p[q]; uint32_t d[4] = {v.x, v.y, v.z, v.w};
                for (int k = 0; k < 4; k++) for (int bb = 0; bb < 4; bb++) m |= (unsigned long long)((d[k] >> (8 * bb)) & 1u) << (q * 16 + k * 4 + bb);
                if ((v.x | v.y | v.z | v.w) & 0x01010101u) p[q] = make_uint4(v.x & 0xfefefefeu, v.y & 0xfefefefeu, v.z & 0xfefefefeu, v.w & 0xfefefefeu);
            }
            contMask[w] = m;
        } else m = contMask[w];
        c = (uint32_t)__popcll(m);
    }
    part[threadIdx.x] = c;
    __syncthreads();
    for (uint32_t off = 1; off < SCAN_WAVES_PER_BLOCK; off <<= 1) { uint32_t v = (threadIdx.x >= off) ? part[threadIdx.x - off] : 0; __syncthreads(); part[threadIdx.x] += v; __syncthreads(); }
    if (w < nW) waveLocal[w] = part[threadIdx.x] - c;
    if (threadIdx.x == SCAN_WAVES_PER_BLOCK - 1) blockSums[blockIdx.x] = part[threadIdx.x];
}
__global__ __launch_bounds__(1024) void k_scan_blocks(const uint32_t* countPtr, uint32_t countImm, uint32_t* blockSums, const uint32_t* waveLocal, uint32_t* nextCount, unsigned long long* tracedRays,
                                                      const unsigned long long* contMask, const uint32_t* curBase , uint32_t Npad, int batch, uint32_t* nextBase,
                                                      uint32_t* hostNextCount, uint32_t* hostNextBase ,
                                                      const uint32_t* activeCount, uint32_t* hostActiveCount )
{
    __shared__ uint32_t part[1024];
    const uint32_t N = countPtr ? *countPtr : countImm;
    const uint32_t nW = (N + 63) / 64, nB = (nW + SCAN_WAVES_PER_BLOCK - 1) / SCAN_WAVES_PER_BLOCK;
    const uint32_t per = (nB + 1023) / 1024;
    const uint32_t t = threadIdx.x;
    uint32_t b = t * per, e = min(b + per, nB);
    uint32_t sum = 0;
    for (uint32_t i = b; i < e; i++) sum += blockSums[i];
    part[t] = sum;
    __syncthreads();
    for (uint32_t off = 1; off < 1024; off <<= 1) { uint32_t v = (t >= off) ? part[t - off] : 0; __syncthreads(); part[t] += v; __syncthreads(); }
    uint32_t run = part[t] - sum;
    for (uint32_t i = b; i < e; i++) { uint32_t c = blockSums[i]; blockSums[i] = run; run += c; }
    if (t == 1023) { *nextCount = part[1023]; *hostNextCount = part[1023]; if (tracedRays) atomicAdd(tracedRays, (unsigned long long)part[1023]); }
    if (t == 0 && hostActiveCount) *hostActiveCount = *activeCount;
    __threadfence_block();
    __syncthreads();
    if (t <= (uint32_t)batch) {
        uint32_t g = (t == (uint32_t)batch) ? N : (curBase ? curBase[t] : t * Npad);
        g = min(g, N);
        uint32_t w = g >> 6, l = g & 63;
        uint32_t v = part[1023];
        if (w < nW) v = blockSums[w / SCAN_WAVES_PER_BLOCK] + waveLocal[w] + (uint32_t)__popcll(contMask[w] & ((1ull << l) - 1ull));
        nextBase[t] = v; hostNextBase[t] = v;
    }
}

template <bool FIRST>
__global__ __launch_bounds__(256) void k_compact(const uint32_t* queue, const uint32_t* countPtr, uint32_t countImm, const unsigned long long* contMask, const uint32_t* waveOffsets, const uint32_t* blockBase,
                                                 const uint32_t* keysTmp, uint32_t* queueNext, uint32_t* keysNext)
{
    const uint32_t N = FIRST ? countImm : *countPtr;
    const uint32_t slot = blockIdx.x * blockDim.x + threadIdx.x;
    if (slot >= N) return;
    const uint32_t w = slot >> 6, lane = slot & 63;
    unsigned long long m = contMask[w];
    if ((m >> lane) & 1ull) {
        uint32_t dst = blockBase[w / SCAN_WAVES_PER_BLOCK] + waveOffsets[w] + (uint32_t)__popcll(m & ((1ull << lane) - 1ull));
        queueNext[dst] = FIRST ? slot : queue[slot];
        keysNext[dst] = keysTmp[slot];
    }
}

#define SORT_BLOCK 256
#define SORT_ITEMS 8
#define SORT_TILE (SORT_BLOCK * SORT_ITEMS)
#define SORT_RADIX 128
__global__ __launch_bounds__(SORT_BLOCK) void k_sort_hist(const uint32_t* keys, const uint32_t* countPtr, uint32_t shift, uint32_t* hist , uint32_t numTilesMax)
{
    __shared__ uint32_t h[SORT_RADIX];
    const uint32_t N = *countPtr;
    const uint32_t tile = blockIdx.x;
    if (tile * SORT_TILE >= N) return;
    if (threadIdx.x < SORT_RADIX) h[threadIdx.x] = 0;
    __syncthreads();
    for (int k = 0; k < SORT_ITEMS; k++) { uint32_t i = tile * SORT_TILE + k * SORT_BLOCK + threadIdx.x; if (i < N) atomicAdd(&h[(keys[i] >> shift) & (SORT_RADIX - 1)], 1u); }
    __syncthreads();
    if (threadIdx.x < SORT_RADIX) hist[threadIdx.x * numTilesMax + tile] = h[threadIdx.x];
}
__global__ __launch_bounds__(1024) void k_sort_scan(const uint32_t* countPtr, uint32_t* hist, uint32_t numTilesMax, uint32_t* digitTotals)
{
    __shared__ uint32_t part[1024];
    const uint32_t N = *countPtr;
    const uint32_t nT = (N + SORT_TILE - 1) / SORT_TILE;
    uint32_t* row = hist + (size_t)blockIdx.x * numTilesMax;
    const uint32_t per = (nT + 1023) / 1024;
    const uint32_t t = threadIdx.x;
    const uint32_t b = min(t * per, nT), e = min(b + per, nT);
    uint32_t sum = 0;
    for (uint32_t i = b; i < e; i++) sum += row[i];
    part[t] = sum;
// ... 43 lines not shown
```

### idkengine_amd/csrc/kernels_shade.hpp

```cpp
#pragma once

DEV void write_trace_ready(const DScene& s, const Frame& f, const TraceBufs& tr, uint32_t rid, const RayState& r)
{
    f3 rd = DecodeUnitVec(r.pdx, r.pdy);
    if (f.useTlas || s.instanceCount > 1) {
        tr.rec[4 * (size_t)rid] = make_float4(r.origin.x, r.origin.y, r.origin.z, 0.0f); tr.rec[4 * (size_t)rid + 1] = make_float4(rd.x, rd.y, rd.z, 0.0f);
        if (f.useTlas || f.instTlas) tr.rec[4 * (size_t)rid + 2] = make_float4(1.0f / rd.x, 1.0f / rd.y, 1.0f / rd.z, 0.0f);
        return;
    }
    GpuBlasInstance inst = s.instances[0];
    M34 inv = load_inv_model(s, inst.MeshTransformId);
    f3 lo = xform34(inv, r.origin, 1.0f), ld = xform34(inv, rd, 0.0f);
    const f3 iv = mk3(1.0f / ld.x, 1.0f / ld.y, 1.0f / ld.z);
    const float4* root = s.nodes + 2 * (size_t)s.descs[inst.BlasId].NodeOffset + 2;
    float t1;
    const float rootT = RayBoxIntersect(lo, iv, root[0], root[1], &t1) ? t1 : __builtin_inff();
    const float wantClosest = (__builtin_isfinite(r.throughput.x) && __builtin_isfinite(r.throughput.y) && __builtin_isfinite(r.throughput.z)) ? 0.0f : 1.0f;
    if (wantClosest != 0.0f && tr.oddCount) atomicAdd(tr.oddCount, 1u);
    tr.rec[4 * (size_t)rid] = make_float4(lo.x, lo.y, lo.z, rootT); tr.rec[4 * (size_t)rid + 1] = make_float4(ld.x, ld.y, ld.z, wantClosest);
    tr.rec[4 * (size_t)rid + 2] = make_float4(iv.x, iv.y, iv.z, 0.0f);
}

template <bool VER >
__global__ __launch_bounds__(256) void k_shade_first(DScene s0, Frame f, RayBufs rays, TraceBufs tr, HitBufs hits, const uint32_t* activeList, const uint32_t* activeCount,
                                                     uint8_t* contFlag, uint32_t* seedsAndKeys, int lean ,
                                                     uint32_t* pmList , uint32_t* pmCount)
{
    __shared__ uint32_t waveCont[4]; __shared__ uint32_t blockBase;
    const uint32_t item = blockIdx.x * blockDim.x + threadIdx.x;
    const uint32_t nActive = *activeCount;
    if (blockIdx.x * blockDim.x >= nActive) return;
    const bool live = item < nActive;
    if (!pmList && !live) return;
    bool cont = false; uint32_t rid = 0;
    if (live) {
        rid = activeList[item];
        const uint32_t smp = rid / f.Npad, pix = rid - smp * f.Npad;
        const DScene s = VER ? scene_of_sample(s0, smp) : s0;
        const uint32_t acc = sample_index(f, smp);
        const HitRec hit = load_hit(hits, rid);
        RayState r; uint32_t rng, key = 0;
        if (lean) {
            f2 pd; gen_primary(f, smp, pix, acc, r.origin, pd, rng);
            r.prevIor = 1.0f; r.throughput = splat3(1.0f); r.pdx = pd.x; r.radiance = splat3(0.0f); r.pdy = pd.y;
        } else {
            float4 a = rays.o_ior[rid], b = rays.thr_px[rid], c = rays.rad_py[rid];
            r.origin = mk3(a.x, a.y, a.z); r.prevIor = a.w; r.throughput = mk3(b.x, b.y, b.z); r.pdx = b.w; r.radiance = mk3(c.x, c.y, c.z); r.pdy = c.w;
            rng = seedsAndKeys[rid];
        }
        AovState aov; aov.albedo = splat3(0.0f); aov.normal = splat3(0.0f); aov.newWeight = 1.0f;
        int lx = (int)(pix % (uint32_t)f.W), ly = (int)(pix / (uint32_t)f.W);
        uint32_t gidSeed = first_hit_gid_seed(f.W, f.H, lx, global_row(f, ly));
        f3 rd = DecodeUnitVec(r.pdx, r.pdy);
        cont = ShadeHit<true>(s, f, acc, hit, hit.T != PT_FLOAT_MAX, rd, r, aov, rng, gidSeed, key);
        rays.o_ior[rid] = make_float4(r.origin.x, r.origin.y, r.origin.z, r.prevIor);
        rays.thr_px[rid] = make_float4(r.throughput.x, r.throughput.y, r.throughput.z, r.pdx);
        rays.rad_py[rid] = make_float4(r.radiance.x, r.radiance.y, r.radiance.z, r.pdy);
        if (f.outputAovs) { rays.aovA[rid] = make_float4(aov.albedo.x, aov.albedo.y, aov.albedo.z, aov.newWeight); rays.aovN[rid] = make_float4(aov.normal.x, aov.normal.y, aov.normal.z, 0.0f); }
        seedsAndKeys[rid] = (key & ((1u << IDKPT_SORT_KEY_BITS) - 1u)) | (smp << IDKPT_SORT_KEY_BITS);
        if (cont) { contFlag[rid] = (uint8_t)(CF_CONTINUES | (f.markLast ? CF_LAST_ENTERED : 0)); write_trace_ready(s, f, tr, rid, r); }
    }
    if (pmList) {
        const unsigned long long m = __ballot(cont);
        const uint32_t wv = threadIdx.x >> 6, lane = threadIdx.x & 63;
        if (lane == 0) waveCont[wv] = (uint32_t)__popcll(m);
        __syncthreads();
        if (threadIdx.x == 0) { uint32_t tot = 0; for (int i = 0; i < 4; i++) { const uint32_t c = waveCont[i]; waveCont[i] = tot; tot += c; } blockBase = tot ? atomicAdd(pmCount, tot) : 0u; }
        __syncthreads();
        if (cont) pmList[blockBase + waveCont[wv] + (uint32_t)__popcll(m & ((1ull << lane) - 1ull))] = rid;
    }
}

template <bool FIRST, bool VER = false>
__global__ __launch_bounds__(256) void k_shade(DScene s0, Frame f, RayBufs rays, TraceBufs tr, HitBufs hits, const uint32_t* queue, const uint32_t* countPtr, uint32_t countImm,
                                               const uint32_t* qbase, const uint32_t* gbase , unsigned long long* contMask, uint32_t* waveCounts, uint32_t* keysTmp)
{
    const uint32_t N = FIRST ? countImm : *countPtr;
    const uint32_t slot = blockIdx.x * blockDim.x + threadIdx.x;
    if ((slot & ~63u) >= N) return;
    bool cont = false;
    uint32_t key = 0;
    bool inRange = slot < N;
    uint32_t smp = 0, pix = 0, idx = 0;
    if (inRange) {
        idx = FIRST ? slot : queue[slot];
        smp = idx / f.Npad; pix = idx - smp * f.Npad;
        if (FIRST && pix >= (uint32_t)f.W * (uint32_t)f.rows) inRange = false;
    }
    if (inRange) {
        const DScene s = VER ? scene_of_sample(s0, smp) : s0;
        const uint32_t acc = sample_index(f, smp);
        float4 a = rays.o_ior[idx], b = rays.thr_px[idx], c = rays.rad_py[idx];
        const HitRec hit = load_hit(hits, (!FIRST && f.hitsByRid) ? idx : slot);
        if (FIRST && f.g.DoDebugBVHTraversal) {
            rays.o_ior[idx] = make_float4(a.x, a.y, a.z, hits.cost[slot]);
        } else {
            RayState r; r.origin = mk3(a.x, a.y, a.z); r.prevIor = a.w; r.throughput = mk3(b.x, b.y, b.z); r.pdx = b.w; r.radiance = mk3(c.x, c.y, c.z); r.pdy = c.w;
            AovState aov; aov.albedo = splat3(0.0f); aov.normal = splat3(0.0f); aov.newWeight = 1.0f;
            if (!FIRST && f.outputAovs) { float4 aa = rays.aovA[idx], an = rays.aovN[idx]; aov.albedo = mk3(aa.x, aa.y, aa.z); aov.newWeight = aa.w; aov.normal = mk3(an.x, an.y, an.z); }
            uint32_t rng, gidSeed;
            if (FIRST) {
                f3 o2; f2 pd2; gen_primary(f, smp, pix, acc, o2, pd2, rng);
                int lx = (int)(pix % (uint32_t)f.W), ly = (int)(pix / (uint32_t)f.W);
                gidSeed = first_hit_gid_seed(f.W, f.H, lx, global_row(f, ly));
            } else {
                uint32_t gslot = (gbase ? gbase[f.gbBands ? smp * (uint32_t)f.gbStride + ((pix / (uint32_t)f.W) >> f.rowBandLog2) : smp] : 0u) + (slot - qbase[smp]);
                rng = gslot * 4096u + acc;
                gidSeed = gslot;
            }
            f3 rd = DecodeUnitVec(r.pdx, r.pdy);
            bool hitScene = hit.T != PT_FLOAT_MAX;
            cont = ShadeHit<FIRST>(s, f, acc, hit, hitScene, rd, r, aov, rng, gidSeed, key);
            rays.o_ior[idx] = make_float4(r.origin.x, r.origin.y, r.origin.z, r.prevIor);
            rays.thr_px[idx] = make_float4(r.throughput.x, r.throughput.y, r.throughput.z, r.pdx);
            rays.rad_py[idx] = make_float4(r.radiance.x, r.radiance.y, r.radiance.z, r.pdy);
            if (f.outputAovs) { rays.aovA[idx] = make_float4(aov.albedo.x, aov.albedo.y, aov.albedo.z, aov.newWeight); rays.aovN[idx] = make_float4(aov.normal.x, aov.normal.y, aov.normal.z, 0.0f); }
            if (cont && tr.rec) write_trace_ready(s, f, tr, idx, r);
            if (!FIRST && cont && f.markLast) rays.flag[idx] = CF_LAST_ENTERED;
        }
        keysTmp[slot] = (key & ((1u << IDKPT_SORT_KEY_BITS) - 1u)) | (smp << IDKPT_SORT_KEY_BITS);
    }
    unsigned long long m = __ballot(cont);
    if ((threadIdx.x & 63) == 0) contMask[slot >> 6] = m;
    (void)waveCounts;
}

template <bool ALL_HITS , bool VER, bool ODD_ONLY>
__device__ __forceinline__ void shade_last_slot(const DScene& s0, const Frame& f, const RayBufs& rays, const HitBufs& hits, const uint32_t* queue, const uint32_t* qbase, float4* radSave, uint32_t slot)
{
    const uint32_t idx = queue[slot];
    const float4 b = rays.thr_px[idx];
    const bool odd = ALL_HITS || !(__builtin_isfinite(b.x) && __builtin_isfinite(b.y) && __builtin_isfinite(b.z));
    if (ODD_ONLY && !odd) return;
    const HitRec hit = load_hit(hits, f.hitsByRid ? idx : slot);
    const bool miss = hit.T == PT_FLOAT_MAX;
    if (!miss && !odd) return;
    const float4 c = rays.rad_py[idx];
    radSave[slot] = c;
    if (miss) {
        const f3 albedo = SampleSky(s0, DecodeUnitVec(b.w, c.w));
        const f3 rad = mk3(c.x, c.y, c.z) + albedo * mk3(b.x, b.y, b.z);
        rays.rad_py[idx] = make_float4(rad.x, rad.y, rad.z, c.w);
    } else {
        const uint32_t smp = idx / f.Npad;
        const DScene s = VER ? scene_of_sample(s0, smp) : s0;
        const uint32_t acc = sample_index(f, smp);
        const float4 a = rays.o_ior[idx];
        RayState r; r.origin = mk3(a.x, a.y, a.z); r.prevIor = a.w; r.throughput = mk3(b.x, b.y, b.z); r.pdx = b.w; r.radiance = mk3(c.x, c.y, c.z); r.pdy = c.w;
        AovState aov; aov.albedo = splat3(0.0f); aov.normal = splat3(0.0f); aov.newWeight = 1.0f;
        const uint32_t gslot = slot - qbase[smp];
        uint32_t rng = gslot * 4096u + acc, key = 0;
        (void)ShadeHit<false, true>(s, f, acc, hit, true, DecodeUnitVec(b.w, c.w), r, aov, rng, gslot, key);
        rays.rad_py[idx] = make_float4(r.radiance.x, r.radiance.y, r.radiance.z, c.w);
    }
}
template <bool ALL_HITS, bool VER = false>
__global__ __launch_bounds__(256) void k_shade_last(DScene s0, Frame f, RayBufs rays, HitBufs hits, const uint32_t* queue, const uint32_t* countPtr, const uint32_t* qbase,
                                                    float4* radSave, uint32_t* deferCount)
{
    const uint32_t N = *countPtr;
    const uint32_t slot = blockIdx.x * blockDim.x + threadIdx.x;
    if (slot == 0u) *deferCount = N;
    if (slot >= N) return;
    shade_last_slot<ALL_HITS, VER, false>(s0, f, rays, hits, queue, qbase, radSave, slot);
}
__global__ __launch_bounds__(256) void k_shade_last_odd(DScene s0, Frame f, RayBufs rays, HitBufs hits, const uint32_t* queue, const uint32_t* countPtr, const uint32_t* qbase,
                                                        float4* radSave, uint32_t* deferCount, const uint32_t* oddCount)
{
    const uint32_t N = *countPtr;
    const uint32_t first = blockIdx.x * blockDim.x + threadIdx.x;
    if (first == 0u) *deferCount = N;
    if (*oddCount == 0u) return;
    for (unsigned long long slot = first; slot < N; slot += (unsigned long long)gridDim.x * blockDim.x) shade_last_slot<false, false, true>(s0, f, rays, hits, queue, qbase, radSave, (uint32_t)slot);
}
template <bool ALL_HITS>
__global__ __launch_bounds__(256) void k_restore_last(RayBufs rays, HitBufs hits, const uint32_t* queue, const uint32_t* countPtr, const float4* radSave, int hitsByRid, int folded)
{
    const uint32_t slot = blockIdx.x * blockDim.x + threadIdx.x;
    if (slot >= *countPtr) return;
    const uint32_t idx = queue[slot];
    const float4 b = rays.thr_px[idx];
    bool restore = ALL_HITS || !(__builtin_isfinite(b.x) && __builtin_isfinite(b.y) && __builtin_isfinite(b.z));
    if (!restore && !folded) restore = load_hit(hits, hitsByRid ? idx : slot).T == PT_FLOAT_MAX;
    if (restore) rays.rad_py[idx] = radSave[slot];
}
```

### idkengine_amd/csrc/kernels_trace.hpp

```cpp
#pragma once

template <bool COUNT, bool COST>
__global__ __launch_bounds__(WAVE) void k_trace_primary(DScene s, Frame f, RayBufs rays, HitBufs hits, uint32_t N, uint32_t* workCounter, uint64_t* counters)
{
    extern __shared__ uint32_t lds[];
    const int lane = threadIdx.x;
    uint32_t* stk = lds + lane;
    uint32_t nPairs = 0, nTris = 0;
    while (true) {
        uint32_t base = wave_grab(workCounter, WAVE);
        if (base >= N) break;
        uint32_t pix = base + lane;
        if (pix < N) {
            f3 origin; f2 pd; uint32_t seed;
            gen_primary(f, 0u, pix, f.accumulated, origin, pd, seed);
            rays.o_ior[pix] = make_float4(origin.x, origin.y, origin.z, 1.0f);
            rays.thr_px[pix] = make_float4(1.0f, 1.0f, 1.0f, pd.x);
            rays.rad_py[pix] = make_float4(0.0f, 0.0f, 0.0f, pd.y);
            f3 rd = DecodeUnitVec(pd.x, pd.y);
            HitRec hit; float cost;
            TraceRay<COUNT, COST>(s, f, origin, rd, hit, cost, stk, WAVE, nPairs, nTris);
            store_hit(hits, pix, hit.T, hit.bx, hit.by, hit.tri, hit.xform);
            if (COST) hits.cost[pix] = cost;
        }
// ... 96 lines not shown
            if (s.skySize <= 0) cls = 7;
            else if (s.skySize > 1) cls = 8;
            else {
                const float eta = 2.0f * (R / F) + 1e-4f;
                int face = -1; bool same = true;
                for (int i = 0; i < 4; i++) {
                    const float ax = gabs(u[i].x), ay = gabs(u[i].y), az = gabs(u[i].z);
                    int fc = -1;
                    if (ax >= gmax(ay, az) + eta) fc = u[i].x > 0.0f ? 0 : 1;
                    else if (ay >= gmax(ax, az) + eta) fc = u[i].y > 0.0f ? 2 : 3;
                    else if (az >= gmax(ax, ay) + eta) fc = u[i].z > 0.0f ? 4 : 5;
                    if (fc < 0 || (face >= 0 && fc != face)) same = false;
                    face = fc;
                }
                if (same && face >= 0) cls = (uint8_t)(1 + face);
            }
        }
    }
    tileClass[(size_t)smp * (tilesX * tilesY) + t] = cls;
}

template <bool VER>
__global__ __launch_bounds__(1024) void k_gen_primary(DScene s0, Frame f, RayBufs rays, TraceBufs tr, int cull, uint32_t* activeList, uint32_t* activeCount, uint32_t* seedOut, uint8_t* contFlag,
                                                     const uint8_t* tileClass ,
                                                     int lean )
{
    __shared__ uint32_t waveKeep[16]; __shared__ uint32_t blockBase; __shared__ unsigned long long keepMask[16];
    const bool pm = f.genPixelMajor != 0;
    if (pm && tileClass && blockIdx.y < ((uint32_t)f.W + 7) / 8 * (((uint32_t)f.rows + 7) / 8) && tileClass[blockIdx.y] != 0u) return;
    const uint32_t G = blockDim.x >> 6;
    const uint32_t smp = pm ? blockIdx.x * G + (threadIdx.x >> 6) : blockIdx.x;
    const DScene s = VER ? scene_of_sample(s0, min(smp, (uint32_t)f.batch - 1u)) : s0;
    const uint32_t wave = pm ? blockIdx.y : (blockIdx.y * blockDim.x + threadIdx.x) >> 6, lane = threadIdx.x & 63;
    const uint32_t tilesX = ((uint32_t)f.W + 7) / 8;
    const uint32_t tx = wave % tilesX, ty = wave / tilesX;
    const uint32_t x = tx * 8 + (lane & 7), y = ty * 8 + (lane >> 3);
    const bool valid = x < (uint32_t)f.W && y < (uint32_t)f.rows && smp < (uint32_t)f.batch;
    const uint32_t pix = y * (uint32_t)f.W + x;
    const uint32_t rid = smp * f.Npad + pix;
    bool keep = false;
    const uint32_t nTilesAll = tilesX * (((uint32_t)f.rows + 7) / 8);
    const uint32_t cls = (tileClass && wave < nTilesAll) ? tileClass[(f.tilePerSample ? (size_t)min(smp, (uint32_t)f.batch - 1u) * nTilesAll : 0) + wave] : 0u;
    if (valid && cls != 0u) {
        contFlag[rid] = CF_CULLED_TILE;
    } else if (valid) {
        f3 origin; f2 pd; uint32_t seed;
        gen_primary(f, smp, pix, sample_index(f, smp), origin, pd, seed);
        f3 rd = DecodeUnitVec(pd.x, pd.y);
        f3 lo = origin, ld = rd, invDir = splat3(0.0f);
        float rootT = __builtin_inff();
        keep = !cull;
        if (f.useTlas || f.instTlas) {
            invDir = mk3(1.0f / rd.x, 1.0f / rd.y, 1.0f / rd.z);
            if (cull) {
                if (s.tlasCount == 0) keep = false;
                else {
                    const uint32_t packed = __float_as_uint(s.tlas[0].w), id = packed & 0x7fffffffu;
                    if ((packed >> 31) == 1u) keep = true;
                    else {
                        float t1, t2;
                        const bool tl = RayBoxIntersect(origin, invDir, s.tlas[2 * (size_t)id], s.tlas[2 * (size_t)id + 1], &t1) && t1 < PT_FLOAT_MAX;
                        const bool tr2 = RayBoxIntersect(origin, invDir, s.tlas[2 * (size_t)id + 2], s.tlas[2 * (size_t)id + 3], &t2) && t2 < PT_FLOAT_MAX;
                        keep = tl || tr2;
                    }
                }
            }
        } else
        for (int ii = 0; ii < s.instanceCount && (ii == 0 || cull); ii++) {
            GpuBlasInstance inst = s.instances[ii];
            M34 inv = load_inv_model(s, inst.MeshTransformId);
            f3 l0 = xform34(inv, origin, 1.0f), l1 = xform34(inv, rd, 0.0f);
            f3 iv = mk3(1.0f / l1.x, 1.0f / l1.y, 1.0f / l1.z);
            if (s.instanceCount == 1) { lo = l0; ld = l1; invDir = iv; }
            if (cull || s.instanceCount == 1) {
                const float4* root = s.nodes + 2 * (size_t)s.descs[inst.BlasId].NodeOffset + 2;
                float t1;
                const bool boxHit = RayBoxIntersect(l0, iv, root[0], root[1], &t1);
                if (s.instanceCount == 1 && boxHit) rootT = t1;
                if (cull && boxHit && t1 < PT_FLOAT_MAX) keep = true;
            }
// ... 299 lines not shown
                        const float t = __int_as_float(__builtin_amdgcn_ds_bpermute(from, __float_as_int(pt)));
                        const float by = __int_as_float(__builtin_amdgcn_ds_bpermute(from, __float_as_int(pby))), bz = __int_as_float(__builtin_amdgcn_ds_bpermute(from, __float_as_int(pbz)));
                        if (k < cnt && j < 64u && t < hitT) {
                            hitTri = leafFirst + k + (MULTI ? triOff : triOffset); hbx = 1.0f - by - bz; hby = by; hitT = t; hitXform = MULTI ? xformId : inst.MeshTransformId;
                            if (OCCL && occl) top = 0u;
                        }
                    }
                    __builtin_amdgcn_wave_barrier();
                    if (base + 64u >= total) leafPending = false;
                }
            }
        }
        if (leafPending) {
            const uint32_t tOff = MULTI ? triOff : triOffset;
            for (uint32_t i = leafFirst + tOff, e = leafEnd + tOff; i < e; i++) {
                const float4* tv = s.triVerts + 3 * (size_t)i + (VER ? vTri : 0u);
                float4 a = tv[0], b = tv[1], c = tv[2];
                float by, bz, t;
                if (RayTriangleIntersect(ro, rd, mk3(a.x, a.y, a.z), mk3(b.x, b.y, b.z), mk3(c.x, c.y, c.z), &by, &bz, &t) && t < hitT) {
                    hitTri = i; hbx = 1.0f - by - bz; hby = by; hitT = t; hitXform = MULTI ? xformId : inst.MeshTransformId;
                    if (OCCL && occl) { top = 0u; break; }
                    if (ANY) {
                        top = 0u; sp = stkBase;
                        if (MULTI) { instIdx = (uint32_t)s.instanceCount; moreInst = false; }
                        break;
                    }
                }
            }
            leafPending = false;
        }
        PROF_MARK(2);
        if (active && top == 0u && (!MULTI || (TLAS ? !moreInst : instIdx >= (uint32_t)s.instanceCount))) {
            if (OCCL && occl && f.foldLast) { if (hitT == PT_FLOAT_MAX) rays.flag[slot] = (uint8_t)(CF_LAST_ENTERED | CF_LAST_MISSED); }
            else store_hit(hits, slot, hitT, hbx, hby, hitTri, hitXform);
            active = false;
        }
    }
    if (ovf) *s.overflow = 1u;
    if (COUNT) flush_counters(counters, nPairs, nTris);
    if (PROF && lane == 0) { for (int i = 0; i < 4; i++) atomicAdd((unsigned long long*)&counters[4 + i], pc[i]); for (int i = 0; i < 8; i++) atomicAdd((unsigned long long*)&counters[8 + i], pn[i]); }
#undef PROF_MARK
}
```

### idkengine_amd/csrc/kernels_trace_fused.hpp

```cpp
#pragma once

template <int REFILL_MIN = 32>
__global__ __launch_bounds__(WAVE, 1) void k_trace_fused(DScene s, Frame f, RayBufs rays, TraceBufs tr, HitBufs hits, const uint32_t* list, const uint32_t* countPtr, uint32_t* workCounter,
                                                        uint8_t* contFlag, uint32_t* seedsAndKeys, int lean)
{
    extern __shared__ uint32_t lds[];
    const uint32_t lane = threadIdx.x;
    typedef __attribute__((address_space(3))) uint32_t lds_u32;
    lds_u32* const stkBase = (lds_u32*)lds + lane;
    const int cap = f.stackCap;
    lds_u32* const stkFull = stkBase + cap * WAVE;
    const uint32_t N = *countPtr;
    {
        uint32_t want = gridDim.x;
        if (f.gridRaysX4 > 0u) want = max((uint32_t)(((unsigned long long)N * 4ull / f.gridRaysX4 + 63ull) / 64ull), min(want, 1024u));
        if (f.gridMid > 0u && N < f.gridMidRays) want = min(want, f.gridMid);
        if (blockIdx.x >= max(want, 1u)) return;
    }
    const GpuBlasInstance inst = s.instances[0];
    const int nodeOffset = s.descs[inst.BlasId].NodeOffset;
    const uint32_t triOffset = (uint32_t)s.descs[inst.BlasId].TriangleOffset;
    const float4* nodes = s.nodes + 2 * (size_t)nodeOffset;

    bool active = false, leafPending = false, workLeft = true;
// ... 86 lines not shown
                float4 a = tv[0], b = tv[1], c = tv[2];
                float by, bz, t;
                if (RayTriangleIntersect(ro, rd, mk3(a.x, a.y, a.z), mk3(b.x, b.y, b.z), mk3(c.x, c.y, c.z), &by, &bz, &t) && t < hitT) {
                    hitTri = i; hbx = 1.0f - by - bz; hby = by; hitT = t; hitXform = inst.MeshTransformId;
                }
            }
            leafPending = false;
        }
        if (active && top == 0u) {
            if (bounce) store_hit(hits, rid, hitT, hbx, hby, hitTri, hitXform);
            else shadePend = true;
            active = false;
        }
        {
            const uint32_t nS = (uint32_t)__builtin_popcountll(__builtin_amdgcn_ballot_w64(shadePend)), nA = (uint32_t)__builtin_popcountll(__builtin_amdgcn_ballot_w64(active));
            if (nS == 0u || !(nS >= (uint32_t)f.shadeMin || nS >= nA)) continue;
        }
        if (shadePend) {
            shadePend = false;
            const uint32_t smp = rid / f.Npad, pix = rid - smp * f.Npad;
            const uint32_t acc = sample_index(f, smp);
            HitRec hit; hit.T = hitT; hit.bx = hbx; hit.by = hby; hit.tri = hitTri; hit.xform = hitXform;
            RayState r; uint32_t rng, key = 0;
            if (lean) {
                f2 pd; gen_primary(f, smp, pix, acc, r.origin, pd, rng);
                r.prevIor = 1.0f; r.throughput = splat3(1.0f); r.pdx = pd.x; r.radiance = splat3(0.0f); r.pdy = pd.y;
            } else {
                float4 a = rays.o_ior[rid], b = rays.thr_px[rid], c = rays.rad_py[rid];
                r.origin = mk3(a.x, a.y, a.z); r.prevIor = a.w; r.throughput = mk3(b.x, b.y, b.z); r.pdx = b.w; r.radiance = mk3(c.x, c.y, c.z); r.pdy = c.w;
                rng = seedsAndKeys[rid];
            }
            AovState aov; aov.albedo = splat3(0.0f); aov.normal = splat3(0.0f); aov.newWeight = 1.0f;
            const int lx = (int)(pix % (uint32_t)f.W), ly = (int)(pix / (uint32_t)f.W);
            const uint32_t gidSeed = first_hit_gid_seed(f.W, f.H, lx, global_row(f, ly));
            const f3 rd0 = DecodeUnitVec(r.pdx, r.pdy);
            const bool cont = ShadeHit<true>(s, f, acc, hit, hit.T != PT_FLOAT_MAX, rd0, r, aov, rng, gidSeed, key);
            rays.o_ior[rid] = make_float4(r.origin.x, r.origin.y, r.origin.z, r.prevIor);
            rays.thr_px[rid] = make_float4(r.throughput.x, r.throughput.y, r.throughput.z, r.pdx);
            rays.rad_py[rid] = make_float4(r.radiance.x, r.radiance.y, r.radiance.z, r.pdy);
            if (f.outputAovs) { rays.aovA[rid] = make_float4(aov.albedo.x, aov.albedo.y, aov.albedo.z, aov.newWeight); rays.aovN[rid] = make_float4(aov.normal.x, aov.normal.y, aov.normal.z, 0.0f); }
            seedsAndKeys[rid] = (key & ((1u << IDKPT_SORT_KEY_BITS) - 1u)) | (smp << IDKPT_SORT_KEY_BITS);
            if (cont) {
                contFlag[rid] = CF_CONTINUES;
                const f3 wd = DecodeUnitVec(r.pdx, r.pdy);
                const M34 inv = load_inv_model(s, inst.MeshTransformId);
                ro = xform34(inv, r.origin, 1.0f); rd = xform34(inv, wd, 0.0f);
                invDir = mk3(1.0f / rd.x, 1.0f / rd.y, 1.0f / rd.z);
                const float4* root = s.nodes + 2 * (size_t)nodeOffset + 2;
                float t1;
                const float rootT = RayBoxIntersect(ro, invDir, root[0], root[1], &t1) ? t1 : __builtin_inff();
                hitT = PT_FLOAT_MAX; hitTri = ~0u; hitXform = 0; hbx = 0.0f; hby = 0.0f;
                if (f.g.DoTraceLights) {
                    for (int i = 0; i < s.lightCount; i++) {
                        const GpuLight& l = s.lights[i];
                        float tMin, tMax;
                        if (RaySphereIntersect(r.origin, wd, mk3(l.Position[0], l.Position[1], l.Position[2]), l.Radius, &tMin, &tMax) && tMin < hitT) { hitT = tMin < 0.0f ? tMax : tMin; hitXform = (uint32_t)i; hitTri = ~0u; }
                    }
                }
                const bool enter = rootT < hitT;
                active = true; bounce = true; leafPending = false; sp = stkBase; top = enter ? 2u : 0u;
            }
        }
    }
    if (ovf) *s.overflow = 1u;
}
```

### idkengine_amd/csrc/pt_kernels.hpp

```cpp
#pragma once
#include "pt_device.hpp"

namespace ptd {

struct TexDesc { const void* data; int w, h; uint32_t state; uint32_t pad; };

struct DScene {
    const float4* nodes;
    const float4* pairNodes;
    const uint4* tris;
    const float4* triVerts;
    const GpuBlasDesc* descs;
    const GpuBlasInstance* instances; int instanceCount;
    const float4* tlas; int tlasCount;
    const float4* instRec;
    const uint4* vertices;
    const GpuMesh* meshes;
    const GpuMaterial* materials;
    const float4* xforms;
    const GpuLight* lights; int lightCount;
    const float4* sky; int skySize;
    const TexDesc* textures; int textureCount;
    const float* srgbLut;
    uint32_t* overflow;
    const uint32_t* ver;
};
#define SCENE_VER_WORDS 8
DEV DScene scene_of_sample(const DScene& s, uint32_t smp)
{
    DScene v = s;
    const uint32_t* t = s.ver + SCENE_VER_WORDS * (size_t)smp;
    v.nodes = s.nodes + t[0]; v.triVerts = s.triVerts + t[1]; v.vertices = s.vertices + t[2]; v.tlas = s.tlas + t[3]; v.xforms = s.xforms + t[4];
    return v;
}

struct Frame {
    float invProj[16]; float invView[16]; float viewPos[3];
    int W, H, rowMod, rowRem, rows;
    int rowBandLog2;
    GpuSettings g;
    uint32_t accumulated;
    int useTlas, stackCap, outputAovs;
    int tlasCap;
    int leafMin;
    uint32_t gridRaysX4, gridMid, gridMidRays;
    int grabUnitLog2, grabFixed;
    int batch; uint32_t Npad; uint32_t accum[256];
    uint32_t seqFirst, seqStride;
    const float* cams; uint32_t slotOf[256];
    int advMin;
    int poolMin;
    int splitPeek;
    int splitMode;
    int scatterLog2;
    int gbStride, gbBands;
    int queryMode;
    int shadeMin;
    int hitsByRid;
    int genPixelMajor;
    int instSieve;
    int instTlas;
    int packet;
    int tilePerSample;
    int markLast;
    int foldLast;
};
enum : uint8_t {
    CF_CONTINUES = 1,
    CF_CULLED_PIXEL = 2,
    CF_CULLED_TILE = 4,
    CF_LAST_ENTERED = 8,
    CF_LAST_MISSED = 16,
};
#define MAX_BATCH 256

struct RayBufs {
    float4* o_ior;
    float4* thr_px;
    float4* rad_py;
    float4* aovA;
    float4* aovN;
    uint8_t* flag;
};
struct TraceBufs {
    float4* rec;
    const uint32_t* order; const uint32_t* orderIdx;
    uint32_t* oddCount;
};
struct HitBufs {
    float4* hit;
    float* cost;
};

struct HitRec { float T, bx, by; uint32_t tri, xform; };
DEV void store_hit(const HitBufs& h, size_t slot, float T, float bx, float by, uint32_t tri, uint32_t xform)
{
    h.hit[2 * slot] = make_float4(T, bx, by, __uint_as_float(tri));
    h.hit[2 * slot + 1] = make_float4(__uint_as_float(xform), 0.0f, 0.0f, 0.0f);
}
DEV HitRec load_hit(const HitBufs& h, size_t slot)
{
    const float4 a = h.hit[2 * slot]; const float x = h.hit[2 * slot + 1].x;
    HitRec r; r.T = a.x; r.bx = a.y; r.by = a.z; r.tri = __float_as_uint(a.w); r.xform = __float_as_uint(x);
    return r;
}

#define TLAS_STACK_SIZE 32

template <bool COUNT, bool COST>
DEV bool IntersectBlas(const DScene& s, f3 ro, f3 rd, const GpuBlasDesc& dref, bool useTlas, HitRec& hit, float& debugCost,
                       uint32_t* stk, int stride, int cap, uint32_t& nPairs, uint32_t& nTris)
{
    bool anyHit = false;
    float tMinLeft, tMinRight;
    f3 invDir = mk3(1.0f / rd.x, 1.0f / rd.y, 1.0f / rd.z);
    struct { int NodeOffset, TriangleOffset; } d = {dref.NodeOffset, dref.TriangleOffset};
    const float4* nodes = s.nodes + 2 * (size_t)d.NodeOffset;
    if (!useTlas) {
        float4 rmin = nodes[2], rmax = nodes[3];
        if (!(RayBoxIntersect(ro, invDir, rmin, rmax, &tMinLeft) && tMinLeft < hit.T)) return false;
    }
    int sp = 0;
    uint32_t top = 2;
    while (true) {
        if (COST) debugCost += 1.0f;
        if (COUNT) nPairs++;
        const float4* p = nodes + 2 * (size_t)top;
        float4 lmin = p[0], lmax = p[1], rmin = p[2], rmax = p[3];
        uint32_t lStart = __float_as_uint(lmin.w), lCount = __float_as_uint(lmax.w), rStart = __float_as_uint(rmin.w), rCount = __float_as_uint(rmax.w);
        bool hitLeft = RayBoxIntersect(ro, invDir, lmin, lmax, &tMinLeft) && tMinLeft <= hit.T;
        bool hitRight = RayBoxIntersect(ro, invDir, rmin, rmax, &tMinRight) && tMinRight <= hit.T;
        bool intersectLeft = hitLeft && lCount > 0, intersectRight = hitRight && rCount > 0;
        if (intersectLeft || intersectRight) {
            uint32_t first = intersectLeft ? lStart : rStart;
            uint32_t end = !intersectRight ? (lStart + lCount) : (rStart + rCount);
            first += (uint32_t)d.TriangleOffset; end += (uint32_t)d.TriangleOffset;
// ... 163 lines not shown
            uint32_t id = packed & 0x7fffffffu;
            if (isLeaf) {
                GpuBlasInstance inst = s.instances[id];
                M34 inv = load_inv_model(s, inst.MeshTransformId);
                f3 lo = xform34(inv, ro, 1.0f), ld = xform34(inv, rd, 0.0f);
                if (IntersectBlasAny(s, lo, ld, s.descs[inst.BlasId], true, hit, stk, stride, f.stackCap)) { hit.xform = inst.MeshTransformId; return true; }
                if (sp == 0 || sp > f.tlasCap) break;
                top = tstk[--sp * stride];
                continue;
            }
            uint32_t l = id, r = id + 1;
            float4 lmin = s.tlas[2 * (size_t)l], lmax = s.tlas[2 * (size_t)l + 1], rmin = s.tlas[2 * (size_t)r], rmax = s.tlas[2 * (size_t)r + 1];
            bool tl = RayBoxIntersect(ro, invDir, lmin, lmax, &tMinLeft) && tMinLeft < hit.T;
            bool tr = RayBoxIntersect(ro, invDir, rmin, rmax, &tMinRight) && tMinRight < hit.T;
            if (tl || tr) {
                if (tl && tr) { bool lc = tMinLeft < tMinRight; top = lc ? l : r; if (sp < f.tlasCap) tstk[sp * stride] = lc ? r : l; else *s.overflow = 1u; sp++; }
                else top = tl ? l : r;
            } else { if (sp == 0 || sp > f.tlasCap) break; top = tstk[--sp * stride]; }
        }
    } else {
        for (int i = 0; i < s.instanceCount; i++) {
            GpuBlasInstance inst = s.instances[i];
            M34 inv = load_inv_model(s, inst.MeshTransformId);
            f3 lo = xform34(inv, ro, 1.0f), ld = xform34(inv, rd, 0.0f);
            if (IntersectBlasAny(s, lo, ld, s.descs[inst.BlasId], false, hit, stk, stride, f.stackCap)) { hit.xform = inst.MeshTransformId; return true; }
        }
    }
    return false;
}

DEV int global_row(const Frame& f, int ly) { return ((((ly >> f.rowBandLog2) * f.rowMod + f.rowRem) << f.rowBandLog2) | (ly & ((1 << f.rowBandLog2) - 1))); }

DEV uint32_t sample_index(const Frame& f, uint32_t smp) { return f.seqFirst + f.accum[smp] * f.seqStride; }
DEV void gen_primary(const Frame& f, uint32_t smp, uint32_t pix, uint32_t acc, f3& origin, f2& packedDir, uint32_t& rngSeed)
{
    const float* cam = f.cams ? f.cams + 36u * smp : f.invProj;
    const float* invProj = cam; const float* invView = cam + 16; const float* vp = cam + 32;
    int lx = (int)(pix % (uint32_t)f.W), ly = (int)(pix / (uint32_t)f.W);
    int y = global_row(f, ly), x = lx;
    uint32_t seed = (uint32_t)(y * 4096 + x) * (acc + 1u);
    float ox = rnd01(seed), oy = rnd01(seed);
    float nx = ((float)x + ox) / (float)f.W * 2.0f - 1.0f, ny = ((float)y + oy) / (float)f.H * 2.0f - 1.0f;
    f3 camDir = GetWorldSpaceDirection(invProj, invView, nx, ny);
    f3 viewPos = mk3(vp[0], vp[1], vp[2]);
    f3 focalPoint = viewPos + camDir * f.g.FocalLength;
    f2 disk = SampleDisk(seed);
    f3 pointOnLense = mat4_mul_xyz(invView, f.g.LenseRadius * disk.x, f.g.LenseRadius * disk.y, 0.0f, 1.0f);
    camDir = normalize(focalPoint - pointOnLense);
    origin = pointOnLense;
    packedDir = EncodeUnitVec(camDir);
    rngSeed = seed;
}

DEV uint32_t first_hit_gid_seed(int W, int H, int px, int py)
{
    const uint32_t n = 20;
    uint32_t numX = (uint32_t)(W + 7) / 8, numY = (uint32_t)(H + 7) / 8;
    uint32_t sx = (uint32_t)px / 8, sy = (uint32_t)py / 8;
    uint32_t columnSize = numY * n, fullColumnCount = numX / n, lastColumnWidth = numX % n;
    uint32_t columnIdx = sx / n;
    uint32_t columnWidth = (columnIdx == fullColumnCount) ? lastColumnWidth : n;
    uint32_t idxInColumn = sy * columnWidth + (sx - columnIdx * n);
    uint32_t idx = columnIdx * columnSize + idxInColumn;
    uint32_t wgY = idx / numX, wgX = idx % numX;
    uint32_t gx = wgX * 8 + (uint32_t)px % 8, gy = wgY * 8 + (uint32_t)py % 8;
    return gy * 4096u + gx;
}

DEV int tex_wrap(int i, int n, uint32_t mode)
{
    if (mode == 1u) return i < 0 ? 0 : (i > n - 1 ? n - 1 : i);
    if (mode == 2u) { int m = i % (2 * n); if (m < 0) m += 2 * n; const int a = m - n; return (n - 1) - (a >= 0 ? a : -(1 + a)); }
    int k = i % n; if (k < 0) k += n; return k;
}
DEV float4 tex_fetch(const DScene& s, const TexDesc& t, int x, int y)
{
    const uint32_t fmt = t.state >> 5;
    const size_t at = (size_t)y * (size_t)t.w + (size_t)x;
    if (fmt == 0u) return ((const float4*)t.data)[at];
    const uint32_t p = ((const uint32_t*)t.data)[at];
    const float a = (float)(p >> 24) / 255.0f;
    if (fmt == 1u) return make_float4((float)(p & 255u) / 255.0f, (float)((p >> 8) & 255u) / 255.0f, (float)((p >> 16) & 255u) / 255.0f, a);
    return make_float4(s.srgbLut[p & 255u], s.srgbLut[(p >> 8) & 255u], s.srgbLut[(p >> 16) & 255u], a);
}
DEV float4 SampleTex(const DScene& s, uint64_t handle, float u, float v)
{
    if (handle == 0 || handle > (uint64_t)s.textureCount) return make_float4(1.0f, 1.0f, 1.0f, 1.0f);
    const TexDesc t = s.textures[handle - 1];
    if (t.w == 1 && t.h == 1) return tex_fetch(s, t, 0, 0);
    const uint32_t ws = t.state & 3u, wt = (t.state >> 2) & 3u;
    if ((t.state >> 4) & 1u) {
        const int x = tex_wrap((int)gfloor(u * (float)t.w), t.w, ws), y = tex_wrap((int)gfloor(v * (float)t.h), t.h, wt);
        return tex_fetch(s, t, x, y);
    }
    float fx = u * (float)t.w - 0.5f, fy = v * (float)t.h - 0.5f;
    float x0f = gfloor(fx), y0f = gfloor(fy);
    float ax = fx - x0f, ay = fy - y0f;
// ... 236 lines not shown
```

### idkengine_amd/gputypes.py

```python
import ctypes as C
import numpy as np

GpuBlasNode = np.dtype([("Min", "<f4", 3), ("TriStartOrChild", "<u4"), ("Max", "<f4", 3), ("TriCount", "<u4")])
GpuBlasTriangle = np.dtype([("X", "<u4"), ("Y", "<u4"), ("Z", "<u4"), ("MeshId", "<u4")])
GpuBlasDesc = np.dtype([
    ("NodeOffset", "<i4"), ("NodeCount", "<i4"), ("TriangleOffset", "<i4"), ("TriangleCount", "<i4"),
    ("LeafIndicesOffset", "<i4"), ("LeafIndicesCount", "<i4"), ("ParentIndicesOffset", "<i4"), ("ParentIndicesCount", "<i4"),
    ("RequiredStackSize", "<i4"), ("IsRefittable", "u1"), ("_pad", "u1", 3)])
GpuBlasInstance = np.dtype([("BlasId", "<u4"), ("MeshTransformId", "<u4")])
GpuTlasNode = np.dtype([("Min", "<f4", 3), ("IsLeafAndChildOrInstanceId", "<u4"), ("Max", "<f4", 3), ("_pad0", "<f4")])
GpuMeshTransform = np.dtype([("Model", "<f4", (3, 4)), ("InvModel", "<f4", (3, 4)), ("PrevModel", "<f4", (3, 4))])
GpuMesh = np.dtype([
    ("LocalBoundsMin", "<f4", 3), ("MaterialId", "<i4"), ("LocalBoundsMax", "<f4", 3), ("NormalMapStrength", "<f4"),
    ("AbsorbanceBias", "<f4", 3), ("MeshletsOffset", "<i4"), ("MeshletCount", "<i4"), ("EmissiveBias", "<f4"),
    ("SpecularBias", "<f4"), ("RoughnessBias", "<f4"), ("TransmissionBias", "<f4"), ("IORBias", "<f4"),
    ("InstanceCount", "<i4"), ("VertexCount", "<i4"), ("_pad0", "<f4", 3), ("TintOnTransmissive", "u1"), ("_pad1", "u1", 3)])
GpuMaterial = np.dtype([
    ("EmissiveFactor", "<f4", 3), ("BaseColorFactor", "<u4"), ("Absorbance", "<f4", 3), ("IOR", "<f4"),
    ("TransmissionFactor", "<f4"), ("RoughnessFactor", "<f4"), ("MetallicFactor", "<f4"), ("AlphaCutoff", "<f4"),
    ("BaseColorTexture", "<u8"), ("MetallicRoughnessTexture", "<u8"), ("NormalTexture", "<u8"), ("EmissiveTexture", "<u8"),
    ("TransmissionTexture", "<u8"), ("IsVolumetric", "u1"), ("_pad0", "u1", 3), ("IsDoubleSided", "u1"), ("_pad1", "u1", 3)])
GpuVertex = np.dtype([("TexCoord", "<f4", 2), ("Tangent", "<u4"), ("Normal", "<u4")])
GpuLight = np.dtype([("Position", "<f4", 3), ("Radius", "<f4"), ("Color", "<f4", 3), ("PointShadowIndex", "<i4"),
                     ("PrevPosition", "<f4", 3), ("_pad0", "<f4")])
# ... 171 lines not shown
class Noise(C.Structure):
    _fields_ = [("Epsilon", C.c_float), ("Threshold", C.c_float)]

    def __init__(self, Epsilon=1e-2, Threshold=0.05):
        super().__init__(float(Epsilon), float(Threshold))


class NoiseSummary(C.Structure):
    _fields_ = [("TilesAbove", C.c_uint32), ("MaxTileMean", C.c_float), ("Tiles", C.c_uint32), ("Samples", C.c_uint32)]


IDKPT_NO_HISTORY = -2
IDKPT_DENOISE_INPUT_ACCUMULATED, IDKPT_DENOISE_INPUT_TEMPORAL = 0, 1


class Reproject(C.Structure):
    _fields_ = [("PrevProjView", C.c_float * 16), ("PrevViewPos", C.c_float * 3), ("PositionTolerance", C.c_float), ("MaxHistory", C.c_float)]

    def __init__(self, PrevProjView=None, PrevViewPos=(0.0, 0.0, 0.0), PositionTolerance=0.02, MaxHistory=32.0):
        m = np.eye(4, dtype=np.float32) if PrevProjView is None else np.asarray(PrevProjView, np.float32)
        super().__init__((C.c_float * 16)(*m.reshape(16).tolist()), (C.c_float * 3)(*[float(v) for v in PrevViewPos]), float(PositionTolerance), float(MaxHistory))

    @classmethod
    def from_camera(cls, cam, **kw):
        return cls((cam.view @ cam.proj).astype(np.float32), cam.position, **kw)


class Stats(C.Structure):
    _fields_ = [("RaysTraced", C.c_uint64), ("PrimaryRays", C.c_uint64), ("Frames", C.c_uint64),
                ("LastAliveCounts", C.c_uint32 * 16), ("LastTraceMs", C.c_float), ("LastFrameMs", C.c_float),
                ("NodePairVisits", C.c_uint64), ("TriangleTests", C.c_uint64),
                ("TraceMsTotal", C.c_double), ("TraceLaunches", C.c_uint64),
                ("WideFlaggedRays", C.c_uint64), ("WideNodeVisits", C.c_uint64), ("WideLeafRecords", C.c_uint64), ("WideTriangleTests", C.c_uint64), ("InstTlasFlaggedRays", C.c_uint64),
                ("PacketFlaggedRays", C.c_uint64), ("PacketPackets", C.c_uint64), ("PacketNodeSteps", C.c_uint64), ("PacketLiveLanes", C.c_uint64), ("PacketRaysEntered", C.c_uint64), ("PacketTriangleRounds", C.c_uint64), ("InstUnifiedLaunches", C.c_uint64), ("InstUnifiedEntries", C.c_uint32), ("InstUnifiedTopDepth", C.c_uint32), ("LastOcclusionLaunches", C.c_uint64), ("LastFoldBatches", C.c_uint64)]


def _ptr(a):
    return None if a is None or len(a) == 0 else a.ctypes.data


class Scene:

    def __init__(self):
        self.blas_nodes = np.zeros(0, GpuBlasNode)
        self.blas_triangles = np.zeros(0, GpuBlasTriangle)
        self.blas_descs = np.zeros(0, GpuBlasDesc)
        self.blas_instances = np.zeros(0, GpuBlasInstance)
        self.tlas_nodes = np.zeros(0, GpuTlasNode)
        self.blas_parent_indices = np.zeros(0, np.int32)
        self.blas_leaf_indices = np.zeros(0, np.int32)
        self.vertex_positions = np.zeros((0, 3), np.float32)
        self.vertices = np.zeros(0, GpuVertex)
        self.meshes = np.zeros(0, GpuMesh)
        self.materials = np.zeros(0, GpuMaterial)
        self.mesh_transforms = np.zeros(0, GpuMeshTransform)
        self.lights = np.zeros(0, GpuLight)
        self.sky_faces = None
        self.textures = []
        self.blas_stack_size = 0

    def desc(self):
        keep = []

        def c(a, dt=None):
            a = np.ascontiguousarray(a, dtype=dt)
            keep.append(a)
            return a
# ... 73 lines not shown
```

### idkengine_amd/pathtracer.py

```python
import ctypes as C
import os
import numpy as np
from . import _lib
from . import gputypes as T
from ._lib import IdkPtError


_OPTION_NAMES = ("force_generic", "no_tile_cull", "no_lean_primary", "leaf_min", "grab_unit_log2", "grab_fixed", "lds_pad", "trace_waves", "grid_hint", "grid_rays_x4", "grid_mid_waves", "defer_last", "last_occlusion", "fold_last", "split", "split_donor", "split_peek", "group_threads", "query_scheduler", "split_scatter", "fused", "fused_shade_min", "leaf_pool", "pool_min", "adv_min",
                 "wide", "wide_cap", "wide_count", "packet", "packet_min_live", "packet_waves", "inst_tlas", "inst_tlas_overlap", "inst_braid", "inst_unify", "inst_unify_radius", "uni_refill", "inst_general", "pair_nodes", "inst_sieve", "inst_sieve_overlap", "gen_pixel_major", "gen_group_max", "bounce_pixel_major", "transport", "bvh_timing", "bvh_small", "bvh_stackopt_host", "force_no_peer", "download_member", "trace_variant")


class PathTracer:
    def __init__(self, width, height, settings=None, device=0, row_modulo=1, row_remainder=0, devices=None, row_band=1):
        self._L = _lib.load()
        n = C.c_int32(0)
        self._L.idkptGetDeviceCount(C.byref(n))
        if n.value <= 0:
            raise IdkPtError("no HIP device visible: the path tracer has no CPU fallback")
        ctx = C.c_void_p()
        ids = list(devices) if devices else [device]
        self.device_count = len(ids); self.device_ids = ids
        if self.device_count > 1 and (row_modulo, row_remainder) != (1, 0):
            raise IdkPtError("a multi-device context deals its rows itself")
        dev = (C.c_int32 * len(ids))(*ids)
        rc = self._L.idkptCreate(len(ids), dev, C.byref(ctx))
        if rc != 0:
            raise IdkPtError(f"idkptCreate failed with status {rc}")
        self._ctx = ctx
        for name in _OPTION_NAMES:
            v = os.environ.get("IDKPT_" + name.upper())
            if v is not None and v != "":
                self.set_option(name, int(v))
        self._settings = settings if settings is not None else T.Settings.default()
        self._cached_ray_depth = self._settings.RayDepth
        self._scene = None
        self.width, self.height = width, height
        self.row_modulo, self.row_remainder, self.row_band = row_modulo, row_remainder, (int(row_band) if row_modulo > 1 else 1)
        self._row_limit = None
        if self.device_count == 1:
            if self.row_band > 1:
                self._check(self._L.idkptSetRowBands(ctx, self.row_band, row_modulo, row_remainder))
# ... 609 lines not shown
        return out

    def temporal_moments_device_ptr(self, slot=None):
        p = C.c_void_p(); n = C.c_size_t()
        self._check(self._L.idkptGetTemporalMomentsDevicePtr(self._ctx, -1 if slot is None else int(slot), C.byref(p), C.byref(n)))
        return p.value, n.value

    def DenoiseTemporal(self, settings=None, slot=None):
        if settings is None:
            settings = T.DenoiseTemporal()
        if not isinstance(settings, T.DenoiseTemporal):
            raise TypeError("DenoiseTemporal: settings must be a gputypes.DenoiseTemporal")
        slot = -1 if slot is None else int(slot)
        self._check(self._L.idkptDenoiseTemporal(self._ctx, slot, C.addressof(settings)))
        return self.DownloadDenoised(slot)

    def enable_counters(self, on=True):
        self._check(self._L.idkptEnableCounters(self._ctx, 1 if on else 0))

    def enable_timing(self, on=True):
        self._check(self._L.idkptEnableTiming(self._ctx, 1 if on else 0))

    def stats(self):
        s = T.Stats()
        self._check(self._L.idkptGetStatsSized(self._ctx, C.addressof(s), C.sizeof(s)))
        return {"rays_traced": s.RaysTraced, "primary_rays": s.PrimaryRays, "frames": s.Frames, "alive_counts": list(s.LastAliveCounts),
                "last_frame_ms": s.LastFrameMs, "node_pair_visits": s.NodePairVisits, "triangle_tests": s.TriangleTests,
                "trace_ms_total": s.TraceMsTotal, "trace_launches": s.TraceLaunches,
                "wide_flagged_rays": s.WideFlaggedRays, "wide_node_visits": s.WideNodeVisits, "wide_leaf_records": s.WideLeafRecords, "wide_triangle_tests": s.WideTriangleTests,
                "inst_tlas_flagged_rays": s.InstTlasFlaggedRays,
                "packet_flagged_rays": s.PacketFlaggedRays, "packet_packets": s.PacketPackets, "packet_node_steps": s.PacketNodeSteps, "packet_live_lanes": s.PacketLiveLanes,
                "packet_rays_entered": s.PacketRaysEntered, "packet_triangle_rounds": s.PacketTriangleRounds,
                "inst_unified_launches": s.InstUnifiedLaunches, "inst_unified_entries": s.InstUnifiedEntries, "inst_unified_top_depth": s.InstUnifiedTopDepth,
                "last_occlusion_launches": s.LastOcclusionLaunches, "last_fold_batches": s.LastFoldBatches}

    def reset_stats(self):
        self._check(self._L.idkptResetStats(self._ctx))

    def image_device_ptr(self, which=0):
        p = C.c_void_p(); n = C.c_size_t()
        self._check(self._L.idkptGetImageDevicePtr(self._ctx, which, C.byref(p), C.byref(n)))
        return p.value, n.value

    def SetFrameRing(self, frames):
        self._check(self._L.idkptSetFrameRing(self._ctx, int(frames)))

    def BeginFrame(self):
        slot = C.c_int32()
        self._check(self._L.idkptBeginFrame(self._ctx, C.byref(slot)))
        return slot.value

    def FrameResult(self, slot, which=0):
        out = np.zeros((self.rows, self.width, 4), np.float32)
        self._check(self._L.idkptDownloadFrame(self._ctx, int(slot), which, out.ctypes.data, out.nbytes))
        return out

    def frame_device_ptr(self, slot, which=0):
        p = C.c_void_p(); n = C.c_size_t()
        self._check(self._L.idkptGetFrameDevicePtr(self._ctx, int(slot), which, C.byref(p), C.byref(n)))
        return p.value, n.value

    def set_max_batch(self, n):
        self._check(self._L.idkptSetMaxBatch(self._ctx, n))

    def flush(self):
        self._check(self._L.idkptFlush(self._ctx))

# ... 6 lines not shown
```

### include/idkpt.h

```cpp
#ifndef IDKPT_H
#define IDKPT_H

#include "idkpt_types.h"

#ifdef __cplusplus
extern "C" {
#endif

#define IDKPT_API __attribute__((visibility("default")))

typedef struct idkpt_ctx idkpt_ctx;

enum idkpt_status {
    IDKPT_OK = 0,
    IDKPT_ERR_UNKNOWN = 1,
    IDKPT_ERR_INVALID_ARGUMENT = 2,
    IDKPT_ERR_INVALID_OPERATION = 3,
    IDKPT_ERR_OUT_OF_MEMORY = 4,
    IDKPT_ERR_NO_DEVICE = 5,
    IDKPT_ERR_HIP = 6,
};

enum idkpt_image { IDKPT_IMAGE_RESULT = 0, IDKPT_IMAGE_ALBEDO = 1, IDKPT_IMAGE_NORMAL = 2 };

// ... 99 lines not shown
    int32_t DoRaySorting;
    int32_t OutputAOVs;
    int32_t UseTlas;
    int32_t BlasStackSize;
} idkpt_settings;

typedef struct idkpt_stats {
    uint64_t RaysTraced;
    uint64_t PrimaryRays;
    uint64_t Frames;
    uint32_t LastAliveCounts[16];
    float    LastTraceMs;
    float    LastFrameMs;
    uint64_t NodePairVisits;
    uint64_t TriangleTests;
    double   TraceMsTotal;
    uint64_t TraceLaunches;
    uint64_t WideFlaggedRays;
    uint64_t WideNodeVisits;
    uint64_t WideLeafRecords;
    uint64_t WideTriangleTests;
    uint64_t InstTlasFlaggedRays;
    uint64_t PacketFlaggedRays;
    uint64_t PacketPackets;
    uint64_t PacketNodeSteps;
    uint64_t PacketLiveLanes;
    uint64_t PacketRaysEntered;
    uint64_t PacketTriangleRounds;
    uint64_t InstUnifiedLaunches;
    uint32_t InstUnifiedEntries;
    uint32_t InstUnifiedTopDepth;
    uint64_t LastOcclusionLaunches;
    uint64_t LastFoldBatches;
} idkpt_stats;
#define IDKPT_ABI_VERSION 13

IDKPT_API int32_t idkptCreate(int32_t deviceCount, const int32_t* deviceIds, idkpt_ctx** outCtx);
IDKPT_API int32_t idkptGetContextDeviceCount(idkpt_ctx* ctx, int32_t* outCount);
enum idkpt_transport { IDKPT_TRANSPORT_NONE = 0, IDKPT_TRANSPORT_PEER_COPY = 1, IDKPT_TRANSPORT_RCCL = 2 };
IDKPT_API int32_t idkptGetTransportInfo(idkpt_ctx* ctx, int32_t* outKind, int32_t* outRanks, int32_t* outRcclVersion, const char** outDetail);
IDKPT_API int32_t idkptTransportSelfTest(int32_t device, int32_t* outRcclVersion, char* outDetail, size_t detailBytes);
enum idkpt_group_sharding { IDKPT_SHARD_AUTO = 0, IDKPT_SHARD_ROWS = 1, IDKPT_SHARD_STRIPS = 2, IDKPT_SHARD_BANDS = 3 };
IDKPT_API int32_t idkptSetGroupSharding(idkpt_ctx* ctx, int32_t mode);
IDKPT_API int32_t idkptDestroy(idkpt_ctx* ctx);
IDKPT_API int32_t idkptGetLastError(idkpt_ctx* ctx, const char** outMessage);
typedef void (*idkpt_error_fn)(void* user, int32_t status, const char* message);
IDKPT_API int32_t idkptSetErrorCallback(idkpt_ctx* ctx, idkpt_error_fn fn, void* user);
IDKPT_API int32_t idkptGetDeviceCount(int32_t* outCount);
IDKPT_API const char* idkptGetVersionString(void);
IDKPT_API int32_t idkptGetAbiVersion(void);

IDKPT_API int32_t idkptSetSize(idkpt_ctx* ctx, int32_t width, int32_t height);
IDKPT_API int32_t idkptSetRowSharding(idkpt_ctx* ctx, int32_t rowModulo, int32_t rowRemainder);
IDKPT_API int32_t idkptSetRowBands(idkpt_ctx* ctx, int32_t bandRows, int32_t rowModulo, int32_t rowRemainder);
IDKPT_API int32_t idkptSetRowRange(idkpt_ctx* ctx, int32_t firstRow, int32_t rowCount);
typedef void (*idkpt_bounce_exchange_fn)(void* user, int32_t bounce, int32_t sampleCount, const uint32_t* localCounts, uint32_t* outBases);
IDKPT_API int32_t idkptSetBounceExchange(idkpt_ctx* ctx, idkpt_bounce_exchange_fn fn, void* user);
typedef void (*idkpt_band_exchange_fn)(void* user, int32_t bounce, int32_t sampleCount, int32_t bandCount, const uint32_t* localCounts, uint32_t* outBases);
IDKPT_API int32_t idkptSetBandExchange(idkpt_ctx* ctx, idkpt_band_exchange_fn fn, void* user);
typedef void (*idkpt_band_exchange_device_fn)(void* user, int32_t bounce, int32_t sampleCount, int32_t bandCount, const uint32_t* dLocalCounts, uint32_t* dOutBases, void* hipStream);
IDKPT_API int32_t idkptSetBandExchangeDevice(idkpt_ctx* ctx, idkpt_band_exchange_device_fn fn, void* user);
IDKPT_API int32_t idkptSetSettings(idkpt_ctx* ctx, const idkpt_settings* settings);
IDKPT_API int32_t idkptGetSettings(idkpt_ctx* ctx, idkpt_settings* outSettings);
IDKPT_API int32_t idkptSetPerFrame(idkpt_ctx* ctx, const float invProjection[16], const float invView[16], const float viewPos[3]);
IDKPT_API int32_t idkptSetPerFrameData(idkpt_ctx* ctx, const GpuPerFrameData* perFrame);

// ... 166 lines not shown
```

Measured before the change: 8402.

## Add 16-byte primary hit records, lazy first-bounce compaction, and magic-number division

Adds a compact 16-byte hit record path for single-instance primary traces, which stores only one float4 per hit and cuts hit-buffer bandwidth. It also defers the first-bounce compaction scatter so the fold/pm last-bounce shading can index through the scan data directly, skipping the scatter when it is not needed. Integer divisions by width and tile counts are replaced with precomputed multiply-shift dividers. These add code paths with more gating conditions, and the ABI stats struct grows while the ABI version number stays unchanged.

```diff
diff --git a/idkengine_amd/csrc/host_context.hpp b/idkengine_amd/csrc/host_context.hpp
--- a/idkengine_amd/csrc/host_context.hpp
+++ b/idkengine_amd/csrc/host_context.hpp
@@ -145,6 +145,8 @@
     int deferLast = 1;
     int lastOcclusion = 1;
     int foldLast = 1;
+    int hit16 = 1;
+    int lazyCompact = 1;
     int graphProbe = 0;
     int gridMidWaves = 20;
     int gridRaysX4 = 6;
@@ -245,9 +247,11 @@
     bool sceneNested = false;
     bool sceneNoEmission = false;
     struct { bool valid = false, allHits = false; int j = 0, side = 0, B = 0; uint32_t total = 0, Npad = 0;
-             bool occl = false, pm = false, fold = false; const uint32_t* list = nullptr; size_t ldsBytes = 0; uint32_t grid = 0; } defer;
+             bool occl = false, pm = false, fold = false, lazyCompact = false ; const uint32_t* list = nullptr; size_t ldsBytes = 0; uint32_t grid = 0; } defer;
     uint64_t occlLaunches = 0;
     uint64_t foldBatches = 0;
+    uint64_t hit16Launches = 0;
+    uint64_t lazyCompacts = 0;
     DevBuf radSave, deferCount;
     bool countersDirty = true;
     uint32_t* hOverflow = nullptr; uint32_t* dOverflow = nullptr;
diff --git a/idkengine_amd/csrc/host_options.hpp b/idkengine_amd/csrc/host_options.hpp
--- a/idkengine_amd/csrc/host_options.hpp
+++ b/idkengine_amd/csrc/host_options.hpp
@@ -21,6 +21,8 @@
     else if (n == "defer_last") o.deferLast = value != 0;
     else if (n == "last_occlusion") o.lastOcclusion = value != 0;
     else if (n == "fold_last") o.foldLast = value != 0;
+    else if (n == "hit16") o.hit16 = value != 0;
+    else if (n == "lazy_compact") o.lazyCompact = value != 0;
     else if (n == "split") { REQUIRE(value >= 0 && value <= 3, "idkptSetDeveloperOption: split is 0..3"); o.split = value; }
     else if (n == "split_donor") o.splitDonor = value != 0;
     else if (n == "split_peek") o.splitPeek = std::max(1, value);
diff --git a/idkengine_amd/csrc/host_readback.hpp b/idkengine_amd/csrc/host_readback.hpp
--- a/idkengine_amd/csrc/host_readback.hpp
+++ b/idkengine_amd/csrc/host_readback.hpp
@@ -136,7 +136,7 @@
     s.RaysTraced = s.PrimaryRays + c[2];
     if (ctx->wtotals.p) { uint64_t w[16]; HIPC(hipMemcpyAsync(w, ctx->wtotals.p, TOTALS_BYTES, hipMemcpyDeviceToHost, ctx->stream)); HIPC(hipStreamSynchronize(ctx->stream)); s.WideFlaggedRays = w[0]; s.WideNodeVisits = w[1]; s.WideLeafRecords = w[2]; s.WideTriangleTests = w[3]; s.InstTlasFlaggedRays = w[4];
         s.PacketFlaggedRays = w[8]; s.PacketPackets = w[9]; s.PacketNodeSteps = w[10]; s.PacketLiveLanes = w[11]; s.PacketRaysEntered = w[12]; s.PacketTriangleRounds = w[13]; }
-    s.LastOcclusionLaunches = ctx->occlLaunches; s.LastFoldBatches = ctx->foldBatches;
+    s.LastOcclusionLaunches = ctx->occlLaunches; s.LastFoldBatches = ctx->foldBatches; s.PrimaryHit16Launches = ctx->hit16Launches; s.LazyCompactBatches = ctx->lazyCompacts;
     s.InstUnifiedLaunches = ctx->uniLaunches; s.InstUnifiedEntries = ctx->derived.holds(derived::UNI) ? (uint32_t)ctx->derived.uniEntries : 0u; s.InstUnifiedTopDepth = ctx->derived.holds(derived::UNI) ? (uint32_t)ctx->derived.uniDepth : 0u;
     *out = s;
     return IDKPT_OK;
@@ -148,7 +148,7 @@
     HIPC(hipSetDevice(ctx->device));
     FLUSH_KEEP();
     HIPC(hipStreamSynchronize(ctx->stream));
-    memset(&ctx->stats, 0, sizeof(ctx->stats)); ctx->uniLaunches = 0; ctx->occlLaunches = 0; ctx->foldBatches = 0;
+    memset(&ctx->stats, 0, sizeof(ctx->stats)); ctx->uniLaunches = 0; ctx->occlLaunches = 0; ctx->foldBatches = 0; ctx->hit16Launches = 0; ctx->lazyCompacts = 0;
     if (ctx->derived.pkStats.host) memset(ctx->derived.pkStats.host, 0, 64);
     for (int i = 0; i < 6; i++) ctx->derived.pkSeen[i] = 0;
     ctx->evUsed = 0; ctx->traceMsAcc = 0.0; ctx->traceLaunchesAcc = 0;
diff --git a/idkengine_amd/csrc/host_schedule.hpp b/idkengine_amd/csrc/host_schedule.hpp
--- a/idkengine_amd/csrc/host_schedule.hpp
+++ b/idkengine_amd/csrc/host_schedule.hpp
@@ -42,6 +42,12 @@
            && !plan.multiVer && !plan.counting && !ctx->counters && (ctx->opt.traceVariant == 0 || ctx->opt.traceVariant == 100);
 }
 static bool want_fold(const dev_ctx* ctx, bool tookOccl) { return tookOccl && ctx->opt.foldLast != 0; }
+static bool want_hit16(const dev_ctx* ctx, const TracePlan& plan, const Frame& f, const DScene& s, bool split)
+{
+    if (ctx->opt.hit16 == 0 || plan.fused || plan.packetPrimary || !(plan.walk == Walk::Plain || plan.walk == Walk::Fast) || (split && plan.splitOk)) return false;
+    if (s.instanceCount != 1 || f.useTlas || f.instTlas || f.g.DoTraceLights || f.queryMode || f.g.DoDebugBVHTraversal || plan.counting || ctx->counters) return false;
+    return ctx->opt.traceVariant == 0 || ctx->opt.traceVariant == 100;
+}
 static bool may_fold(const dev_ctx* ctx, bool deferLast, bool deferAllHits) { return deferLast && !deferAllHits && ctx->opt.lastOcclusion != 0 && ctx->opt.foldLast != 0; }
 static uint32_t small_launch_grid(uint32_t fullGrid, uint32_t prev, int hintMul, int raysX4, uint32_t midGrid)
 {
@@ -63,6 +69,7 @@
     uint32_t* activeList; uint32_t* activeCount;
     uint32_t* pmList; uint32_t* pmCount; bool pmBounce;
     const uint8_t* tileClass; uint32_t midGrid, traceGrid;
+    bool lazyCompact;
     int side;
 };
 static const int BS = MAX_BATCH + 1;
@@ -76,7 +83,7 @@
     b.counts = ctx->counts.as<uint32_t>(); b.bases = ctx->bases.as<uint32_t>(); b.work = ctx->work.as<uint32_t>(); b.counters = ctx->counters64.as<uint64_t>(); b.hostCounts = ctx->dCountsMirror; b.hostBases = ctx->dBasesMirror;
     b.contMask = ctx->contMask.as<unsigned long long>(); b.waveLocal = ctx->waveCounts.as<uint32_t>(); b.blockSums = ctx->blockSums.as<uint32_t>(); b.keysTmp = ctx->keysTmp.as<uint32_t>();
     b.activeList = ctx->sortVals.as<uint32_t>(); b.activeCount = b.counts + (MAX_DEPTH_SLOTS - 1);
-    b.pmList = nullptr; b.pmCount = b.counts + (MAX_DEPTH_SLOTS - 2); b.pmBounce = false; b.tileClass = nullptr; b.side = 1; b.capturing = false;
+    b.pmList = nullptr; b.pmCount = b.counts + (MAX_DEPTH_SLOTS - 2); b.pmBounce = false; b.tileClass = nullptr; b.side = 1; b.capturing = false; b.lazyCompact = false;
 }
 
 static int bounce_tail(Batch& b, int j, const uint32_t* q, const uint32_t* cnt, const uint32_t* gbase, unsigned long long* traced, bool record, const TraceBufs& tr)
@@ -90,6 +97,17 @@
     return IDKPT_OK;
 }
 
+static void first_compact_scatter(Batch& b)
+{
+    launch(k_compact<true>, dim3(b.gridTotal), dim3(256), 0, b.st, nullptr, nullptr, b.total, b.contMask, b.waveLocal, b.blockSums, b.keysTmp, b.ctx->queue[1].as<uint32_t>(), b.ctx->keys[1].as<uint32_t>());
+}
+static bool want_lazy_compact(const dev_ctx* ctx, const Batch& b)
+{
+    if (ctx->opt.lazyCompact == 0 || !b.fast || b.depth != 2 || !b.pmBounce || b.plan.fused || !b.f.markLast) return false;
+    if (ctx->groupExchange || ctx->exchangeFn || ctx->bandExchangeFn || ctx->bandExchangeDevFn) return false;
+    const bool known = ctx->lastFast && ctx->lastBatch == b.B && ctx->hBases != nullptr; const uint32_t prev = ctx->hBases ? ctx->hBases[(size_t)1 * BS + b.B] : 0u;
+    return want_fold(ctx, want_occlusion(ctx, b.plan, true, want_split(ctx, prev, known, b.B)));
+}
 static int finish_deferred(dev_ctx* ctx)
 {
     if (!ctx->defer.valid) return IDKPT_OK;
@@ -97,6 +115,7 @@
     Batch b; batch_views(ctx, b, ctx->defer.B, ctx->defer.Npad);
     b.side = ctx->defer.side; b.f = ctx->lastFrame; b.f.markLast = 0; b.f.foldLast = 0; b.s = make_dscene_last(ctx); b.multiVer = ctx->lastMulti;
     const uint32_t* q = ctx->queue[b.side].as<uint32_t>(); const uint32_t* cnt = ctx->deferCount.as<uint32_t>();
+    if (ctx->defer.lazyCompact) { first_compact_scatter(b); ctx->defer.lazyCompact = false; }
     if (ctx->defer.occl) {
         const int j = ctx->defer.j;
         if (ctx->countersDirty) HIPC(hipMemsetAsync(b.work, 0, WORK_WORDS * 4, b.st));
@@ -168,6 +187,7 @@
     f.W = ctx->W; f.H = ctx->H; f.rowMod = ctx->rowMod; f.rowRem = ctx->rowRem; f.rows = ctx->rows; f.rowBandLog2 = ctx->rowBandLog2;
     f.g = ctx->st.Gpu; f.useTlas = ctx->st.UseTlas; f.stackCap = std::max(1, ctx->st.BlasStackSize > 0 ? ctx->st.BlasStackSize : ctx->sceneStack);
     f.outputAovs = ctx->st.OutputAOVs; f.batch = B; f.Npad = b.Npad;
+    f.dNpad = make_udiv(f.Npad); f.dW = make_udiv((uint32_t)f.W); f.dNumX = make_udiv(((uint32_t)f.W + 7u) / 8u);
     HIPC(ctx->trRec.ensure((size_t)ctx->maxBatch * b.Npad * 64)); b.tr.rec = ctx->trRec.as<float4>();
     for (int k = 0; k < MAX_BATCH; k++) { f.accum[k] = k < B ? ctx->pending[k].accum : 0u; f.slotOf[k] = (uint32_t)(k < B ? ctx->pending[k].slot : 0); }
     f.seqFirst = ctx->seqFirst; f.seqStride = ctx->seqStride; f.accumulated = f.seqFirst + f.accum[0] * f.seqStride;
@@ -196,7 +216,8 @@
     dev_ctx* ctx = b.ctx; hipStream_t st = b.st;
     launch(k_scan_blocks, dim3(1), dim3(1024), 0, st, nullptr, b.total, b.blockSums, b.waveLocal, b.counts + 1, (unsigned long long*)(1 < b.depth ? b.counters + 2 : nullptr), b.contMask, nullptr, b.Npad, b.B, b.bases + 1 * BS, b.hostCounts + 1, b.hostBases + 1 * BS, b.counts + MAX_DEPTH_SLOTS - 1, b.hostCounts + MAX_DEPTH_SLOTS - 1);
     if (ctx->evBounce) HIPC(hipEventRecord(ctx->evBounce[1], st));
-    launch(k_compact<true>, dim3(b.gridTotal), dim3(256), 0, st, nullptr, nullptr, b.total, b.contMask, b.waveLocal, b.blockSums, b.keysTmp, ctx->queue[1].as<uint32_t>(), ctx->keys[1].as<uint32_t>());
+    b.lazyCompact = want_lazy_compact(ctx, b);
+    if (!b.lazyCompact) first_compact_scatter(b);
     return IDKPT_OK;
 }
 
@@ -222,7 +243,11 @@
     uint32_t grid0 = b.traceGrid;
     if (ctx->opt.gridRaysX4 > 0 && known) grid0 = small_launch_grid(b.traceGrid, ctx->hCounts[MAX_DEPTH_SLOTS - 1], 2, ctx->opt.gridRaysX4, b.midGrid);
     if (b.plan.fused) launch(k_trace_fused<32>, dim3(grid0), dim3(WAVE), b.plan.ldsBytes, st, s, f, b.rays, b.tr, b.hits, b.activeList, b.activeCount, b.work + 0, contFlag, b.keysTmp, lean);
-    else launch_trace2<true>(ctx, b.plan, grid0, st, s, f, b.rays, b.tr, b.hits, b.activeList, b.activeCount, b.work + 0, b.counters, want_split(ctx, ctx->hCounts[MAX_DEPTH_SLOTS - 1], known, B), 0);
+    else {
+        const bool split0 = want_split(ctx, ctx->hCounts[MAX_DEPTH_SLOTS - 1], known, B);
+        f.hit16 = want_hit16(ctx, b.plan, f, s, split0) ? 1 : 0; if (f.hit16) ctx->hit16Launches++;
+        launch_trace2<true>(ctx, b.plan, grid0, st, s, f, b.rays, b.tr, b.hits, b.activeList, b.activeCount, b.work + 0, b.counters, split0, 0);
+    }
     TRACE_T1();
     if (ctx->capturePrimary) { HIPC(ctx->primHit.ensure((size_t)N * 16)); launch(k_capture_primary, dim3((N + 255) / 256), dim3(256), 0, st, b.hits, (size_t)(B - 1) * b.Npad, N, ctx->primHit.as<float4>()); }
     if (!b.plan.fused) {
@@ -231,6 +256,7 @@
         if (b.pmBounce) { HIPC(ctx->pmList.ensure((size_t)b.total * 4)); b.pmList = ctx->pmList.as<uint32_t>(); }
         with_flag(b.multiVer, [&](auto VER) { launch(k_shade_first<VER>, dim3(b.gridTotal), dim3(256), 0, st, s, f, b.rays, b.tr, b.hits, b.activeList, b.activeCount, contFlag, b.keysTmp, lean, b.pmList, VER ? nullptr : b.pmCount); });
     }
+    f.hit16 = 0;
     launch(k_scan_local<true>, dim3(b.scanBlocks), dim3(SCAN_WAVES_PER_BLOCK), 0, st, nullptr, b.total, contFlag, b.contMask, b.waveLocal, b.blockSums);
     return first_hit_compact(b);
 }
@@ -309,12 +335,13 @@
 static bool trace_bounce(Batch& b, int j, const uint32_t* q, const uint32_t* cnt, bool readsOnlyHitOrMiss)
 {
     dev_ctx* ctx = b.ctx; hipStream_t st = b.st; const int B = b.B;
-    TRACE_T0();
     const bool known = ctx->lastFast && ctx->lastBatch == B && ctx->hBases != nullptr; const uint32_t prev = ctx->hBases ? ctx->hBases[(size_t)j * BS + B] : 0u;
     uint32_t gridj = b.traceGrid;
     const bool split = want_split(ctx, prev, known, B), occl = b.fast && want_occlusion(ctx, b.plan, readsOnlyHitOrMiss, split);
     if (occl) ctx->occlLaunches++;
     if (want_fold(ctx, occl)) { b.f.foldLast = 1; b.f.hitsByRid = 1; }
+    if (b.lazyCompact && !(b.f.foldLast && b.pmBounce && j == 1)) { first_compact_scatter(b); b.lazyCompact = false; }
+    TRACE_T0();
     if (ctx->opt.gridHint > 0 && ctx->lastBatch == B && ctx->hBases) gridj = small_launch_grid(b.traceGrid, ctx->hBases[(size_t)j * BS + B], ctx->opt.gridHint, ctx->opt.gridRaysX4, b.midGrid);
     if (b.fast && ((b.pmBounce && j == 1) || b.f.foldLast)) {
         const bool pm = b.pmBounce && j == 1;
@@ -332,10 +359,13 @@
     const bool fold = b.f.foldLast != 0, pm = b.pmBounce && j == 1;
     HIPC(ctx->radSave.ensure((size_t)ctx->maxBatch * ctx->Npad * 16));
     auto shade_last = [&](auto ALL, auto VER) { launch(k_shade_last<ALL, VER>, dim3(b.gridTotal), dim3(256), 0, b.st, b.s, b.f, b.rays, b.hits, q, cnt, b.bases + j * BS, ctx->radSave.as<float4>(), ctx->deferCount.as<uint32_t>()); };
-    if (fold) launch(k_shade_last_odd, dim3(std::min<uint32_t>(b.gridTotal, 256u)), dim3(256), 0, b.st, b.s, b.f, b.rays, b.hits, q, cnt, b.bases + j * BS, ctx->radSave.as<float4>(), ctx->deferCount.as<uint32_t>(), (const uint32_t*)b.tr.oddCount);
+    if (fold) launch(k_shade_last_odd, dim3(std::min<uint32_t>(b.gridTotal, 256u)), dim3(256), 0, b.st, b.s, b.f, b.rays, b.hits, q, cnt, b.bases + j * BS, ctx->radSave.as<float4>(), ctx->deferCount.as<uint32_t>(), (const uint32_t*)b.tr.oddCount,
+                     b.lazyCompact ? (const uint32_t*)b.pmList : nullptr, (const uint32_t*)b.pmCount, (const unsigned long long*)b.contMask, (const uint32_t*)b.waveLocal, (const uint32_t*)b.blockSums);
     else if (allHits) with_flag(b.multiVer, [&](auto VER) { shade_last(std::true_type{}, VER); });
     else shade_last(std::false_type{}, std::false_type{});
     if (fold) ctx->foldBatches++;
+    if (b.lazyCompact) ctx->lazyCompacts++;
+    ctx->defer.lazyCompact = b.lazyCompact;
     ctx->defer.allHits = allHits; ctx->defer.valid = true; ctx->defer.j = j; ctx->defer.side = b.side; ctx->defer.B = b.B; ctx->defer.total = b.total; ctx->defer.Npad = b.Npad;
     ctx->defer.occl = occl; ctx->defer.fold = fold; ctx->defer.pm = pm || fold; ctx->defer.list = pm ? (const uint32_t*)b.pmList : q; ctx->defer.ldsBytes = b.plan.ldsBytes; ctx->defer.grid = b.traceGrid;
     return IDKPT_OK;
diff --git a/idkengine_amd/csrc/idkpt_api.hpp b/idkengine_amd/csrc/idkpt_api.hpp
--- a/idkengine_amd/csrc/idkpt_api.hpp
+++ b/idkengine_amd/csrc/idkpt_api.hpp
@@ -997,7 +997,7 @@
         sum.RaysTraced += s.RaysTraced; sum.PrimaryRays += s.PrimaryRays; sum.NodePairVisits += s.NodePairVisits; sum.TriangleTests += s.TriangleTests;
         sum.WideFlaggedRays += s.WideFlaggedRays; sum.WideNodeVisits += s.WideNodeVisits; sum.WideLeafRecords += s.WideLeafRecords; sum.WideTriangleTests += s.WideTriangleTests; sum.InstTlasFlaggedRays += s.InstTlasFlaggedRays;
         sum.PacketFlaggedRays += s.PacketFlaggedRays; sum.PacketPackets += s.PacketPackets; sum.PacketNodeSteps += s.PacketNodeSteps; sum.PacketLiveLanes += s.PacketLiveLanes; sum.PacketRaysEntered += s.PacketRaysEntered; sum.PacketTriangleRounds += s.PacketTriangleRounds;
-        sum.LastOcclusionLaunches += s.LastOcclusionLaunches; sum.LastFoldBatches += s.LastFoldBatches;
+        sum.LastOcclusionLaunches += s.LastOcclusionLaunches; sum.LastFoldBatches += s.LastFoldBatches; sum.PrimaryHit16Launches += s.PrimaryHit16Launches; sum.LazyCompactBatches += s.LazyCompactBatches;
         sum.InstUnifiedLaunches += s.InstUnifiedLaunches; if (d == 0) { sum.InstUnifiedEntries = s.InstUnifiedEntries; sum.InstUnifiedTopDepth = s.InstUnifiedTopDepth; }
         for (int j = 0; j < 16; j++) sum.LastAliveCounts[j] += s.LastAliveCounts[j];
         sum.LastFrameMs = std::max(sum.LastFrameMs, s.LastFrameMs); sum.LastTraceMs = std::max(sum.LastTraceMs, s.LastTraceMs);
diff --git a/idkengine_amd/csrc/kernels_frame.hpp b/idkengine_amd/csrc/kernels_frame.hpp
--- a/idkengine_amd/csrc/kernels_frame.hpp
+++ b/idkengine_amd/csrc/kernels_frame.hpp
@@ -21,7 +21,7 @@
     if (f.outputAovs) { float4 oa = imgAlbedo[(size_t)slot * N + i], on = imgNormal[(size_t)slot * N + i]; ra = mk3(oa.x, oa.y, oa.z); rn = mk3(on.x, on.y, on.z); }
     float m1 = 0.0f, m2 = 0.0f;
     if constexpr (NOISE) { const float4 om = imgMoments[(size_t)slot * momStride + i]; m1 = om.x; m2 = om.y; }
-    const uint32_t px = i % (uint32_t)f.W, py = i / (uint32_t)f.W, tilesX = ((uint32_t)f.W + 7) / 8;
+    uint32_t px, py; udivmod(i, f.dW, py, px); const uint32_t tilesX = f.dNumX.d;
     const uint32_t tile = (py >> 3) * tilesX + (px >> 3), nTilesAll = tilesX * (((uint32_t)f.rows + 7) / 8);
     const uint32_t sharedCls = (tileClass && !f.tilePerSample) ? tileClass[tile] : 0u;
     for (int k = 0; k < f.batch; k++) {
@@ -51,7 +51,7 @@
         else if (cls <= 6u) { const float4 p = s.sky[cls - 1u]; nr = splat3(0.0f) + mk3(p.x, p.y, p.z) * splat3(1.0f); }
         else if (cls == 8u) {
             f3 origin; f2 pd; uint32_t seed;
-            gen_primary(f, (uint32_t)k, i, sample_index(f, (uint32_t)k), origin, pd, seed);
+            gen_primary(f, (uint32_t)k, (int)px, (int)py, sample_index(f, (uint32_t)k), origin, pd, seed);
             const f3 albedo = SampleSky(s, DecodeUnitVec(pd.x, pd.y));
             nr = splat3(0.0f) + albedo * splat3(1.0f);
         }
@@ -87,14 +87,15 @@
     if (pix >= N) return;
     const size_t rid = (size_t)smp * f.Npad + pix;
     uint8_t flag = contFlag[rid];
+    uint32_t px, py; udivmod(pix, f.dW, py, px);
     if (tileClass) {
-        const uint32_t px = pix % (uint32_t)f.W, py = pix / (uint32_t)f.W, tilesX = ((uint32_t)f.W + 7) / 8, nTilesAll = tilesX * (((uint32_t)f.rows + 7) / 8);
+        const uint32_t tilesX = f.dNumX.d, nTilesAll = tilesX * (((uint32_t)f.rows + 7) / 8);
         if (tileClass[(f.tilePerSample ? (size_t)smp * nTilesAll : 0) + (py >> 3) * tilesX + (px >> 3)] != 0u) flag = CF_CULLED_TILE;
     }
     flag &= (uint8_t)(CF_CULLED_PIXEL | CF_CULLED_TILE);
     if (flag == 0) return;
     f3 origin; f2 pd; uint32_t seed;
-    gen_primary(f, smp, pix, sample_index(f, smp), origin, pd, seed);
+    gen_primary(f, smp, (int)px, (int)py, sample_index(f, smp), origin, pd, seed);
     rays.o_ior[rid] = make_float4(origin.x, origin.y, origin.z, 1.0f);
     rays.thr_px[rid] = make_float4(1.0f, 1.0f, 1.0f, pd.x);
     if (flag == CF_CULLED_TILE) {
diff --git a/idkengine_amd/csrc/kernels_queue.hpp b/idkengine_amd/csrc/kernels_queue.hpp
--- a/idkengine_amd/csrc/kernels_queue.hpp
+++ b/idkengine_amd/csrc/kernels_queue.hpp
@@ -27,7 +27,6 @@
     starts[t] = lo - lo0;
 }
 
-#define SCAN_WAVES_PER_BLOCK 256
 template <bool FROM_FLAGS>
 __global__ __launch_bounds__(SCAN_WAVES_PER_BLOCK) void k_scan_local(const uint32_t* countPtr, uint32_t countImm, uint8_t* contFlag, unsigned long long* contMask, uint32_t* waveLocal, uint32_t* blockSums)
 {
@@ -84,7 +83,7 @@
         g = min(g, N);
         uint32_t w = g >> 6, l = g & 63;
         uint32_t v = part[1023];
-        if (w < nW) v = blockSums[w / SCAN_WAVES_PER_BLOCK] + waveLocal[w] + (uint32_t)__popcll(contMask[w] & ((1ull << l) - 1ull));
+        if (w < nW) v = compact_slot(contMask[w], waveLocal, blockSums, w, l);
         nextBase[t] = v; hostNextBase[t] = v;
     }
 }
@@ -99,7 +98,7 @@
     const uint32_t w = slot >> 6, lane = slot & 63;
     unsigned long long m = contMask[w];
     if ((m >> lane) & 1ull) {
-        uint32_t dst = blockBase[w / SCAN_WAVES_PER_BLOCK] + waveOffsets[w] + (uint32_t)__popcll(m & ((1ull << lane) - 1ull));
+        uint32_t dst = compact_slot(m, waveOffsets, blockBase, w, lane);
         queueNext[dst] = FIRST ? slot : queue[slot];
         keysNext[dst] = keysTmp[slot];
     }
diff --git a/idkengine_amd/csrc/kernels_shade.hpp b/idkengine_amd/csrc/kernels_shade.hpp
--- a/idkengine_amd/csrc/kernels_shade.hpp
+++ b/idkengine_amd/csrc/kernels_shade.hpp
@@ -35,13 +35,15 @@
     bool cont = false; uint32_t rid = 0;
     if (live) {
         rid = activeList[item];
-        const uint32_t smp = rid / f.Npad, pix = rid - smp * f.Npad;
+        uint32_t smp, pix; udivmod(rid, f.dNpad, smp, pix);
+        uint32_t ulx, uly; udivmod(pix, f.dW, uly, ulx);
+        const int lx = (int)ulx, ly = (int)uly;
         const DScene s = VER ? scene_of_sample(s0, smp) : s0;
         const uint32_t acc = sample_index(f, smp);
-        const HitRec hit = load_hit(hits, rid);
+        const HitRec hit = f.hit16 ? load_hit16(hits, rid, (uint32_t)s.instances[0].MeshTransformId) : load_hit(hits, rid);
         RayState r; uint32_t rng, key = 0;
         if (lean) {
-            f2 pd; gen_primary(f, smp, pix, acc, r.origin, pd, rng);
+            f2 pd; gen_primary(f, smp, lx, ly, acc, r.origin, pd, rng);
             r.prevIor = 1.0f; r.throughput = splat3(1.0f); r.pdx = pd.x; r.radiance = splat3(0.0f); r.pdy = pd.y;
         } else {
             float4 a = rays.o_ior[rid], b = rays.thr_px[rid], c = rays.rad_py[rid];
@@ -49,8 +51,7 @@
             rng = seedsAndKeys[rid];
         }
         AovState aov; aov.albedo = splat3(0.0f); aov.normal = splat3(0.0f); aov.newWeight = 1.0f;
-        int lx = (int)(pix % (uint32_t)f.W), ly = (int)(pix / (uint32_t)f.W);
-        uint32_t gidSeed = first_hit_gid_seed(f.W, f.H, lx, global_row(f, ly));
+        uint32_t gidSeed = first_hit_gid_seed(f, lx, global_row(f, ly));
         f3 rd = DecodeUnitVec(r.pdx, r.pdy);
         cont = ShadeHit<true>(s, f, acc, hit, hit.T != PT_FLOAT_MAX, rd, r, aov, rng, gidSeed, key);
         rays.o_ior[rid] = make_float4(r.origin.x, r.origin.y, r.origin.z, r.prevIor);
@@ -84,7 +85,7 @@
     uint32_t smp = 0, pix = 0, idx = 0;
     if (inRange) {
         idx = FIRST ? slot : queue[slot];
-        smp = idx / f.Npad; pix = idx - smp * f.Npad;
+        udivmod(idx, f.dNpad, smp, pix);
         if (FIRST && pix >= (uint32_t)f.W * (uint32_t)f.rows) inRange = false;
     }
     if (inRange) {
@@ -100,11 +101,11 @@
             if (!FIRST && f.outputAovs) { float4 aa = rays.aovA[idx], an = rays.aovN[idx]; aov.albedo = mk3(aa.x, aa.y, aa.z); aov.newWeight = aa.w; aov.normal = mk3(an.x, an.y, an.z); }
             uint32_t rng, gidSeed;
             if (FIRST) {
-                f3 o2; f2 pd2; gen_primary(f, smp, pix, acc, o2, pd2, rng);
-                int lx = (int)(pix % (uint32_t)f.W), ly = (int)(pix / (uint32_t)f.W);
-                gidSeed = first_hit_gid_seed(f.W, f.H, lx, global_row(f, ly));
+                uint32_t ulx, uly; udivmod(pix, f.dW, uly, ulx); const int lx = (int)ulx, ly = (int)uly;
+                f3 o2; f2 pd2; gen_primary(f, smp, lx, ly, acc, o2, pd2, rng);
+                gidSeed = first_hit_gid_seed(f, lx, global_row(f, ly));
             } else {
-                uint32_t gslot = (gbase ? gbase[f.gbBands ? smp * (uint32_t)f.gbStride + ((pix / (uint32_t)f.W) >> f.rowBandLog2) : smp] : 0u) + (slot - qbase[smp]);
+                uint32_t gslot = (gbase ? gbase[f.gbBands ? smp * (uint32_t)f.gbStride + (udiv(pix, f.dW) >> f.rowBandLog2) : smp] : 0u) + (slot - qbase[smp]);
                 rng = gslot * 4096u + acc;
                 gidSeed = gslot;
             }
@@ -126,9 +127,8 @@
 }
 
 template <bool ALL_HITS , bool VER, bool ODD_ONLY>
-__device__ __forceinline__ void shade_last_slot(const DScene& s0, const Frame& f, const RayBufs& rays, const HitBufs& hits, const uint32_t* queue, const uint32_t* qbase, float4* radSave, uint32_t slot)
-{
-    const uint32_t idx = queue[slot];
+__device__ __forceinline__ void shade_last_ray(const DScene& s0, const Frame& f, const RayBufs& rays, const HitBufs& hits, const uint32_t* qbase, float4* radSave, uint32_t slot, uint32_t idx )
+{
     const float4 b = rays.thr_px[idx];
     const bool odd = ALL_HITS || !(__builtin_isfinite(b.x) && __builtin_isfinite(b.y) && __builtin_isfinite(b.z));
     if (ODD_ONLY && !odd) return;
@@ -154,6 +154,11 @@
         rays.rad_py[idx] = make_float4(r.radiance.x, r.radiance.y, r.radiance.z, c.w);
     }
 }
+template <bool ALL_HITS, bool VER, bool ODD_ONLY>
+__device__ __forceinline__ void shade_last_slot(const DScene& s0, const Frame& f, const RayBufs& rays, const HitBufs& hits, const uint32_t* queue, const uint32_t* qbase, float4* radSave, uint32_t slot)
+{
+    shade_last_ray<ALL_HITS, VER, ODD_ONLY>(s0, f, rays, hits, qbase, radSave, slot, queue[slot]);
+}
 template <bool ALL_HITS, bool VER = false>
 __global__ __launch_bounds__(256) void k_shade_last(DScene s0, Frame f, RayBufs rays, HitBufs hits, const uint32_t* queue, const uint32_t* countPtr, const uint32_t* qbase,
                                                     float4* radSave, uint32_t* deferCount)
@@ -165,12 +170,22 @@
     shade_last_slot<ALL_HITS, VER, false>(s0, f, rays, hits, queue, qbase, radSave, slot);
 }
 __global__ __launch_bounds__(256) void k_shade_last_odd(DScene s0, Frame f, RayBufs rays, HitBufs hits, const uint32_t* queue, const uint32_t* countPtr, const uint32_t* qbase,
-                                                        float4* radSave, uint32_t* deferCount, const uint32_t* oddCount)
+                                                        float4* radSave, uint32_t* deferCount, const uint32_t* oddCount,
+                                                        const uint32_t* lazyList , const uint32_t* lazyCount, const unsigned long long* contMask, const uint32_t* waveOffsets, const uint32_t* blockBase)
 {
     const uint32_t N = *countPtr;
     const uint32_t first = blockIdx.x * blockDim.x + threadIdx.x;
     if (first == 0u) *deferCount = N;
     if (*oddCount == 0u) return;
+    if (lazyList) {
+        const uint32_t M = *lazyCount;
+        for (unsigned long long i = first; i < M; i += (unsigned long long)gridDim.x * blockDim.x) {
+            const uint32_t idx = lazyList[i], w = idx >> 6, l = idx & 63u;
+            const uint32_t slot = compact_slot(contMask[w], waveOffsets, blockBase, w, l);
+            shade_last_ray<false, false, true>(s0, f, rays, hits, qbase, radSave, slot, idx);
+        }
+        return;
+    }
     for (unsigned long long slot = first; slot < N; slot += (unsigned long long)gridDim.x * blockDim.x) shade_last_slot<false, false, true>(s0, f, rays, hits, queue, qbase, radSave, (uint32_t)slot);
 }
 template <bool ALL_HITS>
diff --git a/idkengine_amd/csrc/kernels_trace.hpp b/idkengine_amd/csrc/kernels_trace.hpp
--- a/idkengine_amd/csrc/kernels_trace.hpp
+++ b/idkengine_amd/csrc/kernels_trace.hpp
@@ -152,8 +152,8 @@
     const uint32_t smp = pm ? blockIdx.x * G + (threadIdx.x >> 6) : blockIdx.x;
     const DScene s = VER ? scene_of_sample(s0, min(smp, (uint32_t)f.batch - 1u)) : s0;
     const uint32_t wave = pm ? blockIdx.y : (blockIdx.y * blockDim.x + threadIdx.x) >> 6, lane = threadIdx.x & 63;
-    const uint32_t tilesX = ((uint32_t)f.W + 7) / 8;
-    const uint32_t tx = wave % tilesX, ty = wave / tilesX;
+    const uint32_t tilesX = f.dNumX.d;
+    uint32_t tx, ty; udivmod(wave, f.dNumX, ty, tx);
     const uint32_t x = tx * 8 + (lane & 7), y = ty * 8 + (lane >> 3);
     const bool valid = x < (uint32_t)f.W && y < (uint32_t)f.rows && smp < (uint32_t)f.batch;
     const uint32_t pix = y * (uint32_t)f.W + x;
@@ -165,7 +165,7 @@
         contFlag[rid] = CF_CULLED_TILE;
     } else if (valid) {
         f3 origin; f2 pd; uint32_t seed;
-        gen_primary(f, smp, pix, sample_index(f, smp), origin, pd, seed);
+        gen_primary(f, smp, (int)x, (int)y, sample_index(f, smp), origin, pd, seed);
         f3 rd = DecodeUnitVec(pd.x, pd.y);
         f3 lo = origin, ld = rd, invDir = splat3(0.0f);
         float rootT = __builtin_inff();
@@ -531,6 +531,7 @@
         PROF_MARK(2);
         if (active && top == 0u && (!MULTI || (TLAS ? !moreInst : instIdx >= (uint32_t)s.instanceCount))) {
             if (OCCL && occl && f.foldLast) { if (hitT == PT_FLOAT_MAX) rays.flag[slot] = (uint8_t)(CF_LAST_ENTERED | CF_LAST_MISSED); }
+            else if (PRIMARY && !MULTI && f.hit16) store_hit16(hits, slot, hitT, hbx, hby, hitTri);
             else store_hit(hits, slot, hitT, hbx, hby, hitTri, hitXform);
             active = false;
         }
diff --git a/idkengine_amd/csrc/kernels_trace_fused.hpp b/idkengine_amd/csrc/kernels_trace_fused.hpp
--- a/idkengine_amd/csrc/kernels_trace_fused.hpp
+++ b/idkengine_amd/csrc/kernels_trace_fused.hpp
@@ -142,7 +142,7 @@
             }
             AovState aov; aov.albedo = splat3(0.0f); aov.normal = splat3(0.0f); aov.newWeight = 1.0f;
             const int lx = (int)(pix % (uint32_t)f.W), ly = (int)(pix / (uint32_t)f.W);
-            const uint32_t gidSeed = first_hit_gid_seed(f.W, f.H, lx, global_row(f, ly));
+            const uint32_t gidSeed = first_hit_gid_seed(f, lx, global_row(f, ly));
             const f3 rd0 = DecodeUnitVec(r.pdx, r.pdy);
             const bool cont = ShadeHit<true>(s, f, acc, hit, hit.T != PT_FLOAT_MAX, rd0, r, aov, rng, gidSeed, key);
             rays.o_ior[rid] = make_float4(r.origin.x, r.origin.y, r.origin.z, r.prevIor);
diff --git a/idkengine_amd/csrc/pt_kernels.hpp b/idkengine_amd/csrc/pt_kernels.hpp
--- a/idkengine_amd/csrc/pt_kernels.hpp
+++ b/idkengine_amd/csrc/pt_kernels.hpp
@@ -1,5 +1,6 @@
 #pragma once
 #include "pt_device.hpp"
+#include "uniform_div.hpp"
 
 namespace ptd {
 
@@ -63,6 +64,8 @@
     int packet;
     int tilePerSample;
     int markLast;
+    UDiv dNpad, dW, dNumX;
+    int hit16;
     int foldLast;
 };
 enum : uint8_t {
@@ -73,6 +76,11 @@
     CF_LAST_MISSED = 16,
 };
 #define MAX_BATCH 256
+#define SCAN_WAVES_PER_BLOCK 256
+DEV uint32_t compact_slot(unsigned long long m, const uint32_t* waveOffsets, const uint32_t* blockBase, uint32_t w, uint32_t lane)
+{
+    return blockBase[w / SCAN_WAVES_PER_BLOCK] + waveOffsets[w] + (uint32_t)__popcll(m & ((1ull << lane) - 1ull));
+}
 
 struct RayBufs {
     float4* o_ior;
@@ -102,6 +110,13 @@
 {
     const float4 a = h.hit[2 * slot]; const float x = h.hit[2 * slot + 1].x;
     HitRec r; r.T = a.x; r.bx = a.y; r.by = a.z; r.tri = __float_as_uint(a.w); r.xform = __float_as_uint(x);
+    return r;
+}
+DEV void store_hit16(const HitBufs& h, size_t rid, float T, float bx, float by, uint32_t tri) { h.hit[2 * rid] = make_float4(T, bx, by, __uint_as_float(tri)); }
+DEV HitRec load_hit16(const HitBufs& h, size_t rid, uint32_t xform)
+{
+    const float4 a = h.hit[2 * rid];
+    HitRec r; r.T = a.x; r.bx = a.y; r.by = a.z; r.tri = __float_as_uint(a.w); r.xform = xform;
     return r;
 }
 
@@ -331,11 +346,10 @@
 DEV int global_row(const Frame& f, int ly) { return ((((ly >> f.rowBandLog2) * f.rowMod + f.rowRem) << f.rowBandLog2) | (ly & ((1 << f.rowBandLog2) - 1))); }
 
 DEV uint32_t sample_index(const Frame& f, uint32_t smp) { return f.seqFirst + f.accum[smp] * f.seqStride; }
-DEV void gen_primary(const Frame& f, uint32_t smp, uint32_t pix, uint32_t acc, f3& origin, f2& packedDir, uint32_t& rngSeed)
+DEV void gen_primary(const Frame& f, uint32_t smp, int lx, int ly, uint32_t acc, f3& origin, f2& packedDir, uint32_t& rngSeed)
 {
     const float* cam = f.cams ? f.cams + 36u * smp : f.invProj;
     const float* invProj = cam; const float* invView = cam + 16; const float* vp = cam + 32;
-    int lx = (int)(pix % (uint32_t)f.W), ly = (int)(pix / (uint32_t)f.W);
     int y = global_row(f, ly), x = lx;
     uint32_t seed = (uint32_t)(y * 4096 + x) * (acc + 1u);
     float ox = rnd01(seed), oy = rnd01(seed);
@@ -350,18 +364,23 @@
     packedDir = EncodeUnitVec(camDir);
     rngSeed = seed;
 }
-
-DEV uint32_t first_hit_gid_seed(int W, int H, int px, int py)
+DEV void gen_primary(const Frame& f, uint32_t smp, uint32_t pix, uint32_t acc, f3& origin, f2& packedDir, uint32_t& rngSeed)
+{
+    uint32_t lx, ly; udivmod(pix, f.dW, ly, lx);
+    gen_primary(f, smp, (int)lx, (int)ly, acc, origin, packedDir, rngSeed);
+}
+
+DEV uint32_t first_hit_gid_seed(const Frame& f, int px, int py)
 {
     const uint32_t n = 20;
-    uint32_t numX = (uint32_t)(W + 7) / 8, numY = (uint32_t)(H + 7) / 8;
+    uint32_t numX = f.dNumX.d, numY = (uint32_t)(f.H + 7) / 8;
     uint32_t sx = (uint32_t)px / 8, sy = (uint32_t)py / 8;
     uint32_t columnSize = numY * n, fullColumnCount = numX / n, lastColumnWidth = numX % n;
     uint32_t columnIdx = sx / n;
     uint32_t columnWidth = (columnIdx == fullColumnCount) ? lastColumnWidth : n;
     uint32_t idxInColumn = sy * columnWidth + (sx - columnIdx * n);
     uint32_t idx = columnIdx * columnSize + idxInColumn;
-    uint32_t wgY = idx / numX, wgX = idx % numX;
+    uint32_t wgY, wgX; udivmod(idx, f.dNumX, wgY, wgX);
     uint32_t gx = wgX * 8 + (uint32_t)px % 8, gy = wgY * 8 + (uint32_t)py % 8;
     return gy * 4096u + gx;
 }
diff --git a/idkengine_amd/csrc/uniform_div.hpp b/idkengine_amd/csrc/uniform_div.hpp
--- /dev/null
+++ b/idkengine_amd/csrc/uniform_div.hpp
@@ -0,0 +1,37 @@
+#pragma once
+#include <stdint.h>
+
+#if defined(__HIPCC__)
+#define UDIV_HD __host__ __device__ __forceinline__
+#else
+#define UDIV_HD inline
+#endif
+
+struct UDiv { uint32_t d, mul, shift; };
+
+inline UDiv make_udiv(uint32_t d)
+{
+    UDiv r; r.d = d; r.mul = 0u; r.shift = 0u;
+    if (d <= 1u) { r.d = 1u; return r; }
+    uint32_t L = 0; while ((1ull << L) < (uint64_t)d) L++;
+    const uint64_t m = (1ull << (32 + L)) / d + 1ull;
+    r.mul = (uint32_t)(m - (1ull << 32)); r.shift = L;
+    return r;
+}
+
+UDIV_HD uint32_t udiv_mulhi(uint32_t a, uint32_t b)
+{
+#if defined(__HIP_DEVICE_COMPILE__)
+    return __umulhi(a, b);
+#else
+    return (uint32_t)(((uint64_t)a * (uint64_t)b) >> 32);
+#endif
+}
+UDIV_HD uint32_t udiv(uint32_t n, const UDiv& v)
+{
+    const uint32_t t = udiv_mulhi(n, v.mul);
+    const uint32_t s1 = v.shift != 0u ? 1u : 0u;
+    return (t + ((n - t) >> s1)) >> (v.shift - s1);
+}
+UDIV_HD uint32_t umod(uint32_t n, const UDiv& v) { return n - udiv(n, v) * v.d; }
+UDIV_HD void udivmod(uint32_t n, const UDiv& v, uint32_t& q, uint32_t& r) { q = udiv(n, v); r = n - q * v.d; }
diff --git a/idkengine_amd/gputypes.py b/idkengine_amd/gputypes.py
--- a/idkengine_amd/gputypes.py
+++ b/idkengine_amd/gputypes.py
@@ -227,7 +227,7 @@
                 ("NodePairVisits", C.c_uint64), ("TriangleTests", C.c_uint64),
                 ("TraceMsTotal", C.c_double), ("TraceLaunches", C.c_uint64),
                 ("WideFlaggedRays", C.c_uint64), ("WideNodeVisits", C.c_uint64), ("WideLeafRecords", C.c_uint64), ("WideTriangleTests", C.c_uint64), ("InstTlasFlaggedRays", C.c_uint64),
-                ("PacketFlaggedRays", C.c_uint64), ("PacketPackets", C.c_uint64), ("PacketNodeSteps", C.c_uint64), ("PacketLiveLanes", C.c_uint64), ("PacketRaysEntered", C.c_uint64), ("PacketTriangleRounds", C.c_uint64), ("InstUnifiedLaunches", C.c_uint64), ("InstUnifiedEntries", C.c_uint32), ("InstUnifiedTopDepth", C.c_uint32), ("LastOcclusionLaunches", C.c_uint64), ("LastFoldBatches", C.c_uint64)]
+                ("PacketFlaggedRays", C.c_uint64), ("PacketPackets", C.c_uint64), ("PacketNodeSteps", C.c_uint64), ("PacketLiveLanes", C.c_uint64), ("PacketRaysEntered", C.c_uint64), ("PacketTriangleRounds", C.c_uint64), ("InstUnifiedLaunches", C.c_uint64), ("InstUnifiedEntries", C.c_uint32), ("InstUnifiedTopDepth", C.c_uint32), ("LastOcclusionLaunches", C.c_uint64), ("LastFoldBatches", C.c_uint64), ("PrimaryHit16Launches", C.c_uint64), ("LazyCompactBatches", C.c_uint64)]
 
 
 def _ptr(a):
diff --git a/idkengine_amd/pathtracer.py b/idkengine_amd/pathtracer.py
--- a/idkengine_amd/pathtracer.py
+++ b/idkengine_amd/pathtracer.py
@@ -6,7 +6,7 @@
 from ._lib import IdkPtError
 
 
-_OPTION_NAMES = ("force_generic", "no_tile_cull", "no_lean_primary", "leaf_min", "grab_unit_log2", "grab_fixed", "lds_pad", "trace_waves", "grid_hint", "grid_rays_x4", "grid_mid_waves", "defer_last", "last_occlusion", "fold_last", "split", "split_donor", "split_peek", "group_threads", "query_scheduler", "split_scatter", "fused", "fused_shade_min", "leaf_pool", "pool_min", "adv_min",
+_OPTION_NAMES = ("force_generic", "no_tile_cull", "no_lean_primary", "leaf_min", "grab_unit_log2", "grab_fixed", "lds_pad", "trace_waves", "grid_hint", "grid_rays_x4", "grid_mid_waves", "defer_last", "last_occlusion", "fold_last", "hit16", "lazy_compact", "split", "split_donor", "split_peek", "group_threads", "query_scheduler", "split_scatter", "fused", "fused_shade_min", "leaf_pool", "pool_min", "adv_min",
                  "wide", "wide_cap", "wide_count", "packet", "packet_min_live", "packet_waves", "inst_tlas", "inst_tlas_overlap", "inst_braid", "inst_unify", "inst_unify_radius", "uni_refill", "inst_general", "pair_nodes", "inst_sieve", "inst_sieve_overlap", "gen_pixel_major", "gen_group_max", "bounce_pixel_major", "transport", "bvh_timing", "bvh_small", "bvh_stackopt_host", "force_no_peer", "download_member", "trace_variant")
 
 
@@ -682,7 +682,8 @@
                 "packet_flagged_rays": s.PacketFlaggedRays, "packet_packets": s.PacketPackets, "packet_node_steps": s.PacketNodeSteps, "packet_live_lanes": s.PacketLiveLanes,
                 "packet_rays_entered": s.PacketRaysEntered, "packet_triangle_rounds": s.PacketTriangleRounds,
                 "inst_unified_launches": s.InstUnifiedLaunches, "inst_unified_entries": s.InstUnifiedEntries, "inst_unified_top_depth": s.InstUnifiedTopDepth,
-                "last_occlusion_launches": s.LastOcclusionLaunches, "last_fold_batches": s.LastFoldBatches}
+                "last_occlusion_launches": s.LastOcclusionLaunches, "last_fold_batches": s.LastFoldBatches,
+                "primary_hit16_launches": s.PrimaryHit16Launches, "lazy_compact_batches": s.LazyCompactBatches}
 
     def reset_stats(self):
         self._check(self._L.idkptResetStats(self._ctx))
diff --git a/include/idkpt.h b/include/idkpt.h
--- a/include/idkpt.h
+++ b/include/idkpt.h
@@ -155,6 +155,8 @@
     uint32_t InstUnifiedTopDepth;
     uint64_t LastOcclusionLaunches;
     uint64_t LastFoldBatches;
+    uint64_t PrimaryHit16Launches;
+    uint64_t LazyCompactBatches;
 } idkpt_stats;
 #define IDKPT_ABI_VERSION 13
 
```

After: 8558, median of 6. +1.9%, better.
